# rrahn/libspm

Hardware: AMD Instinct MI355X
Metric: Gbases/s scanned, Myers k<=3 |P|=100 (higher is better)
Workload: dtype u32

## Files before the change

### libspm_amd/csrc/common.hpp

```cpp
#pragma once

#include <hip/hip_runtime.h>

#include <algorithm>
#include <cstdint>
#include <functional>
#include <cstdio>
#include <string>
#include <utility>
#include <vector>

#include "../../include/spm_hip.h"
#include "scan_plan.hpp"

namespace spm_hip
{

constexpr int kWave = 64;

struct error_sink
{
    std::string msg;
};

extern thread_local std::string g_init_error;

}

struct hits_block
{
    spm_hit *d_hits = nullptr;
    unsigned long long *d_count = nullptr;
    uint64_t cap = 0;
    hipEvent_t ev[4] = {nullptr, nullptr, nullptr, nullptr};
    bool zeroed = false;
    unsigned long long *h_c = nullptr;
    hipEvent_t ev_done = nullptr;
};

struct spm_ctx
{
    int device = 0;
    hipStream_t stream = nullptr;
    bool own_stream = false;
    int n_cu = 256;
    std::string err;
    void *d_scratch = nullptr;
    size_t scratch_bytes = 0;
    std::vector<hits_block> pool;
    std::vector<std::pair<void *, uint64_t>> jst_pool;
    ulonglong2 *d_band_tab = nullptr;
    uint64_t band_slots = 0;
    bool band_dirty = false;
    uint32_t *d_table_poison = nullptr;
    uint8_t *h_stage = nullptr;
    size_t stage_half = 0;
    hipEvent_t stage_ev[2] = {nullptr, nullptr};
    unsigned long long *h_counters = nullptr;
};

struct spm_text
{
    spm_ctx *ctx = nullptr;
    uint8_t *d = nullptr;
    uint64_t n = 0;
    uint64_t alloc = 0;
    uint32_t sigma = 4;
    bool owned = false;
    uint32_t *d_packed = nullptr;
    uint64_t packed_words = 0;
};

struct spm_hits : hits_block
{
    spm_ctx *ctx = nullptr;
    uint64_t cand_cap = 0;
    uint64_t band_cap = 0;
    uint64_t n = 0;
    bool counted = false;
    bool hook_final = false;
    unsigned long long fan_count = 0;
    bool sorted_host = false;
    std::vector<spm_hit> host;
    spm_scan_stats stats{};
    bool timed = false;
    void *d_aux[2] = {nullptr, nullptr};
    bool pending = false;
    bool c_on_the_way = false;
    bool d_count_cleared = false;
    const spm_text *d_text = nullptr;
    const struct spm_patterns *d_patterns = nullptr;
    uint64_t d_begin = 0, d_end = 0;
    spm_scan_opts d_opts{};
    const spm_text *al_text = nullptr;
    const struct spm_patterns *al_patterns = nullptr;
    uint64_t al_lo = 0;
    uint64_t al_pos_offset = 0;
    bool al_stateful = false;
    bool al_device_segs = false;
    std::vector<uint64_t> al_segs;
};

inline void hits_adopt(spm_hits &h, spm_hits &from)
{
    std::swap(static_cast<hits_block &>(h), static_cast<hits_block &>(from));
    std::swap(h.h_c, from.h_c);
    std::swap(h.ev_done, from.ev_done);
    std::swap(h.d_aux, from.d_aux);
    from.d_count_cleared = h.d_count_cleared;
    h.d_count_cleared = false;
    h.n = from.n;
    h.counted = from.counted;
    h.stats = from.stats;
    h.cand_cap = from.cand_cap;
    h.band_cap = from.band_cap;
    h.timed = from.timed;
    h.sorted_host = false;
    h.host.clear();
}

#define SPM_TRY(call)                                                                                                  \
    do {                                                                                                               \
        const int _rc = (call);                                                                                        \
        if (_rc != SPM_OK)                                                                                             \
            return _rc;                                                                                                \
    } while (0)

struct pass_entry
{
    const uint4 *ht;
    uint32_t ht_mask;
    uint32_t pad;
};

struct dev_scratch
{
    std::vector<void *> owned;
    template <typename T>
    hipError_t alloc(T **p, size_t bytes)
    {
        const hipError_t e = hipMalloc(reinterpret_cast<void **>(p), bytes);
        if (e == hipSuccess)
            owned.push_back(*p);
        return e;
    }
    ~dev_scratch()
    {
        for (void *p : owned)
            hipFree(p);
    }
};

#define SPM_SET_ERR(ctx, ...)                                                                                          \
    do {                                                                                                               \
        char _b[512];                                                                                                  \
        snprintf(_b, sizeof(_b), __VA_ARGS__);                                                                         \
        if (ctx)                                                                                                       \
            (ctx)->err = _b;                                                                                           \
        else                                                                                                           \
            spm_hip::g_init_error = _b;                                                                                \
    } while (0)

#define SPM_HIP_CHECK(ctx, call)                                                                                       \
    do {                                                                                                               \
        hipError_t _e = (call);                                                                                        \
        if (_e != hipSuccess) {                                                                                        \
            SPM_SET_ERR(ctx, "%s failed: %s (%s:%d)", #call, hipGetErrorString(_e), __FILE__, __LINE__);               \
            return SPM_E_HIP;                                                                                          \
        }                                                                                                              \
    } while (0)
```

### libspm_amd/csrc/filter.hpp

```cpp
#pragma once

#include "brute.hpp"
#include "common.hpp"
#include "filter_shared.hpp"
#include "pack.hpp"
#include "hd.hpp"

namespace spm_hip
{

struct survivor
{
    uint32_t key;
    uint32_t t_lo, t_hi;
    uint32_t pad;
};
constexpr uint32_t kSurvInvalid = 0xFFFFFFFFu;

struct band_rec
{
    uint32_t slot;
    uint32_t val;
    uint32_t seg;
    uint32_t band;
// ... 996 lines not shown
        return (uint32_t)(W.hi >> (2 * (first - 32)));
    return (uint32_t)(W.lo >> (2 * first)) | (first ? (uint32_t)(W.hi << (2 * (32 - first)) ) : 0u);
}

__device__ __forceinline__ bool seed_sig_ok(const text64 &W, uint32_t sig, uint32_t r, uint32_t n, uint32_t H)
{
    if (n == 0)
        return true;
    const uint32_t rb = r < 16 ? r : 16;
    const uint32_t nl = rb < n ? rb : n;
    uint32_t got = nl ? syms16(W, 16 - rb) : 0u;
    if (nl < 16) {
        got &= (1u << (2 * nl)) - 1;
        got |= syms16(W, 16 + H) << (2 * nl);
    }
    const uint32_t mask = n >= 16 ? 0xFFFFFFFFu : ((1u << (2 * n)) - 1);
    return ((got ^ sig) & mask) == 0;
}

constexpr uint32_t kPairCap = 128;
struct pair_queue
{
    uint32_t t_lo[kPairCap], t_hi[kPairCap], val[kPairCap], rng[kPairCap], seg[kPairCap];
};
struct band_queue
{
    uint32_t key_lo[kPairCap], key_hi[kPairCap], run_lo[kPairCap], run_hi[kPairCap];
    uint32_t elect[128];
};

struct band_chunk
{
    uint64_t base;
    uint32_t used, size, draws;
};
constexpr uint32_t kDenseDraws = 4;

__device__ __forceinline__ void insert_bands(const resolve_params &R, band_queue &B, uint32_t first, uint32_t n,
                                             uint32_t lane, band_chunk &C)
{
    bool act = lane < n;
    unsigned long long bkey = 0, run = 0;
    if (act)
        bkey = ((unsigned long long)B.key_hi[first + lane] << 32) | B.key_lo[first + lane];
    if (!R.overlap) {
        const uint32_t h = (uint32_t)mix64(bkey) & 127u;
        if (act)
            B.elect[h] = lane;
        __builtin_amdgcn_fence(__ATOMIC_RELEASE, "wavefront");
        __builtin_amdgcn_wave_barrier();
        const uint32_t w = act ? B.elect[h] : lane;
        const unsigned long long wkey = ((unsigned long long)B.key_hi[first + w] << 32) | B.key_lo[first + w];
        const bool follower = act && w != lane && wkey == bkey;
        if (follower) {
            atomicOr(&B.run_lo[first + w], B.run_lo[first + lane]);
            atomicOr(&B.run_hi[first + w], B.run_hi[first + lane]);
            act = false;
        }
        __builtin_amdgcn_fence(__ATOMIC_RELEASE, "wavefront");
        __builtin_amdgcn_wave_barrier();
    }
    if (act)
        run = ((unsigned long long)B.run_hi[first + lane] << 32) | B.run_lo[first + lane];
    bool claimed = false;
    uint32_t s2 = (uint32_t)mix64(bkey) & R.table_mask;
    if (act) {
        bool placed = false;
        for (uint32_t tries = 0; tries < 8192 && !placed; ++tries) {
            if ((tries & 31u) == 31u && __hip_atomic_load(&R.counters[kCntVoid], __ATOMIC_RELAXED, __HIP_MEMORY_SCOPE_AGENT) != 0)
                break;
            const unsigned long long o = atomicCAS(&R.band_tab[s2].x, kBandEmpty, bkey);
            if (o == kBandEmpty) {
                claimed = true;
                placed = true;
            } else if (o == bkey) {
                placed = true;
            } else {
                s2 = (s2 + 1) & R.table_mask;
            }
        }
        if (!placed) {
            atomicAdd(&R.counters[kCntVoid], 1ull);
            *R.table_poison = 1u;
        }
        else if (R.overlap)
            atomicAdd(&R.band_tab[s2].y, 1ull);
        else
            atomicAnd(&R.band_tab[s2].y, ~run);
    }
    const uint64_t mm = __ballot(claimed);
    if (mm == 0)
        return;
    const uint32_t nn = __popcll(mm);
    if (C.used + nn > C.size) {
        for (uint32_t q = C.used + lane; q < C.size; q += 64)
            if (C.base + q < R.band_cap)
                R.bands[C.base + q].val = kBandInvalid;
        uint32_t next = C.size * 2 < kChunkMin ? kChunkMin : (C.size * 2 > kChunkMax ? kChunkMax : C.size * 2);
        next = next < nn ? nn : next;
        if (C.draws < kDenseDraws) {
            next = nn;
            ++C.draws;
        }
        unsigned long long b = 0;
        if (lane == 0)
            b = atomicAdd(&R.counters[kCntBandSlots], (unsigned long long)next);
        C.base = ((uint64_t)(uint32_t)__builtin_amdgcn_readfirstlane((uint32_t)(b >> 32)) << 32) |
                 (uint32_t)__builtin_amdgcn_readfirstlane((uint32_t)b);
        C.used = 0;
        C.size = next;
    }
    if (claimed) {
        const uint64_t idx = C.base + C.used + __popcll(mm & ((1ull << lane) - 1));
        if (idx < R.band_cap) {
            band_rec br;
            br.slot = s2;
            br.val = (uint32_t)(bkey >> 43) << 11;
            br.seg = (uint32_t)((bkey & ((1ull << 43) - 1)) >> R.band_bits);
            br.band = (uint32_t)(bkey & ((1ull << R.band_bits) - 1));
            R.bands[idx] = br;
        } else {
            atomicAdd(&R.counters[kCntVoid], 1ull);
            *R.table_poison = 1u;
        }
    }
    C.used += nn;
}

__device__ __forceinline__ unsigned long long wave_reserve_hits(unsigned long long *counter, uint32_t mine)
{
    const uint32_t lane = threadIdx.x & 63;
    uint32_t incl = mine;
#pragma unroll
    for (int o = 1; o < 64; o <<= 1) {
        const uint32_t up = (uint32_t)__shfl_up((int)incl, o);
        if (lane >= (uint32_t)o)
            incl += up;
    }
    const uint32_t total = (uint32_t)__shfl((int)incl, 63);
    unsigned long long base = 0;
    if (total != 0) {
        if (lane == 0)
            base = atomicAdd(counter, (unsigned long long)total);
        base = ((unsigned long long)(uint32_t)__builtin_amdgcn_readfirstlane((uint32_t)(base >> 32)) << 32) |
               (uint32_t)__builtin_amdgcn_readfirstlane((uint32_t)base);
    }
    return base + (incl - mine);
}

__device__ __forceinline__ bool seen_insert_raw(unsigned long long *seen, uint32_t seen_mask, unsigned long long *overflow,
                                                uint32_t pat, int64_t e)
{
    const unsigned long long key = ((unsigned long long)pat << 40) | (unsigned long long)e;
    uint32_t slot = (uint32_t)(mix64(key)) & seen_mask;
    for (uint32_t tries = 0; tries < 64; ++tries) {
        if (tries == 4 && __hip_atomic_load(overflow, __ATOMIC_RELAXED, __HIP_MEMORY_SCOPE_AGENT) != 0)
            return false;
        const unsigned long long old = atomicCAS(&seen[slot], ~0ull, key);
        if (old == ~0ull)
            return true;
        if (old == key)
            return false;
        slot = (slot + 1) & seen_mask;
    }
    atomicAdd(overflow, 1ull);
    return false;
}

struct resolve_wave
{
    pair_queue *Q;
    band_queue *B;
    uint32_t qn, bn;
    band_chunk C;
    uint32_t n_cand;
};

__device__ __forceinline__ void queue_sync()
{
    __builtin_amdgcn_fence(__ATOMIC_RELEASE, "wavefront");
    __builtin_amdgcn_wave_barrier();
}

__device__ __forceinline__ void check_pairs(const resolve_params &R, resolve_wave &S, uint32_t n, uint32_t lane)
{
    pair_queue &Q = *S.Q;
    band_queue &B = *S.B;
    S.qn -= n;
    const uint32_t first = S.qn;
    bool live = lane < n;
    uint64_t t = 0, seg = 0;
    uint32_t val = 0, rng = 0;
    int64_t sb = (int64_t)R.hay_begin, se = (int64_t)R.hay_end;
    if (live) {
        const uint32_t i = first + lane;
        t = ((uint64_t)Q.t_hi[i] << 32) | Q.t_lo[i];
        val = Q.val[i];
        rng = Q.rng[i];
        seg = Q.seg[i];
        if (R.seg_offsets) {
            sb = (int64_t)R.seg_offsets[seg];
            se = (int64_t)R.seg_offsets[seg + 1];
        }
    }
    queue_sync();
    bool through = live;
    const uint32_t pat = val >> 11;
    if (live && !(rng & kRngRun)) {
        if (!(rng & kSeedChecked)) {
            live = seed_intact(R, t, val, (rng >> 16) & 0x1F, (rng & kRngWhole) ? R.key_len + ((rng >> 5) & 0x1F) : 0u, sb, se);
            rng |= kSeedChecked;
        }
        through = live;
        if (live && R.pieces_check) {
            const uint32_t m = (uint32_t)R.m[pat], k = (uint32_t)R.k[pat];
            if (pieces_apply(R, t, val, m, k, sb, se)) {
                const uint32_t v = pieces_visit(R, t, val, rng, m, k);
                live = v != 0;
                through = v == 2;
            }
        }
    }
    {
        const bool back = live && !through;
        const uint64_t mm = __ballot(back);
        if (back) {
            const uint32_t q = S.qn + __popcll(mm & ((1ull << lane) - 1));
            Q.t_lo[q] = (uint32_t)t;
            Q.t_hi[q] = (uint32_t)(t >> 32);
            Q.val[q] = val;
            Q.rng[q] = rng;
            Q.seg[q] = (uint32_t)seg;
        }
        S.qn += __popcll(mm);
    }
    int64_t b_cur = 0, b_last = -1, d_lo = 0, d_hi = 0;
    if (R.exact_hits) {
        bool fresh = false;
        int64_t e = 0;
        if (live && through) {
            ++S.n_cand;
            e = (int64_t)t - (int64_t)(val & 0x7FF) + (int64_t)R.m[pat];
            int64_t own_b = (int64_t)R.scan_begin, own_e = (int64_t)R.scan_end;
            if (R.seg_offsets) {
                own_b = R.seg_owned ? sb + (int64_t)R.seg_owned[seg] : sb;
                own_e = se;
            }
            fresh = e >= own_b + 1 && e <= own_e && (!R.seen || seen_insert_raw(R.seen, R.seen_mask, R.overflow, pat, e));
        }
        const unsigned long long idx = wave_reserve_hits(R.hit_counter, fresh ? 1u : 0u);
        if (fresh && idx < R.hit_cap) {
            spm_hit h;
            h.pos = (R.report_begin ? (uint64_t)(e - (int64_t)R.m[pat]) : (uint64_t)e) + R.pos_offset;
            h.pattern = pat;
            h.score = 0;
            R.hits[idx] = h;
        }
        queue_sync();
        return;
    }
    if (live && through) {
        ++S.n_cand;
        d_hi = (int64_t)t - (int64_t)(val & 0x7FF) - sb + (int64_t)R.max_m;
        d_lo = d_hi - (int64_t)((rng & kRngRun) ? (rng & 0x7FF) : 0u);
        b_cur = d_lo / (int64_t)R.Bw;
        b_last = d_hi / (int64_t)R.Bw;
        if (R.overlap && b_cur > 0 && d_lo - b_cur * (int64_t)R.Bw <= (int64_t)R.k[pat])
            --b_cur;
        if ((uint64_t)b_last >> R.band_bits) {
            atomicAdd(&R.counters[kCntVoid], 1ull);
            b_last = b_cur - 1;
        }
    }
    for (;;) {
        const bool have = b_cur <= b_last;
        const uint64_t mm = __ballot(have);
        if (mm == 0)
            break;
        if (have) {
            const unsigned long long bkey =
                ((unsigned long long)pat << 43) | ((unsigned long long)seg << R.band_bits) | (unsigned long long)b_cur;
            const int64_t b0 = b_cur * (int64_t)R.Bw;
            const uint32_t o_lo = (uint32_t)(d_lo > b0 ? d_lo - b0 : 0);
            const uint32_t o_hi = (uint32_t)(d_hi < b0 + (int64_t)R.Bw - 1 ? d_hi - b0 : (int64_t)R.Bw - 1);
            const unsigned long long run = (o_hi - o_lo >= 63 ? ~0ull : ((1ull << (o_hi - o_lo + 1)) - 1)) << o_lo;
            const uint32_t q = S.bn + __popcll(mm & ((1ull << lane) - 1));
            B.key_lo[q] = (uint32_t)bkey;
            B.key_hi[q] = (uint32_t)(bkey >> 32);
            B.run_lo[q] = (uint32_t)run;
            B.run_hi[q] = (uint32_t)(run >> 32);
        }
        S.bn += __popcll(mm);
        queue_sync();
        if (S.bn >= 64) {
            S.bn -= 64;
            insert_bands(R, B, S.bn, 64, lane, S.C);
            queue_sync();
        }
        ++b_cur;
    }
    queue_sync();
}

__global__ __launch_bounds__(256) void resolve_kernel(const resolve_params R)
{
    __shared__ pair_queue pair_queues[4];
    __shared__ band_queue band_queues[4];
    unsigned long long n = R.counters[kCntSurvSlots];
    if (blockIdx.x == 0 && threadIdx.x == 0) {
        atomicAdd(&R.counters[kCntUnreadSurvSum], n);
        atomicMax(&R.counters[kCntUnreadSurvMax], n);
    }
    if (n > R.surv_cap)
        n = R.surv_cap;
    if (!R.exact_hits && __hip_atomic_load(R.table_poison, __ATOMIC_RELAXED, __HIP_MEMORY_SCOPE_AGENT) != 0) {
        if (blockIdx.x == 0 && threadIdx.x == 0)
            atomicAdd(&R.counters[kCntVoid], 1ull);
        return;
    }
    const uint32_t lane = threadIdx.x & 63;
    resolve_wave S;
    S.Q = &pair_queues[threadIdx.x >> 6];
    S.B = &band_queues[threadIdx.x >> 6];
    S.qn = 0;
    S.bn = 0;
    S.C.base = 0;
    S.C.used = 0;
    S.C.size = 0;
    S.C.draws = 0;
    S.n_cand = 0;
    pair_queue &Q = *S.Q;
    const uint64_t stride = (uint64_t)gridDim.x * blockDim.x;
    const uint64_t rounds = (n + stride - 1) / stride;
    for (uint64_t r = 0; r < rounds; ++r) {
        if ((r & 7u) == 7u &&
            __builtin_amdgcn_readfirstlane((uint32_t)(__hip_atomic_load(&R.counters[kCntVoid], __ATOMIC_RELAXED, __HIP_MEMORY_SCOPE_AGENT) != 0)))
            break;
        const uint64_t i = r * stride + (uint64_t)blockIdx.x * blockDim.x + threadIdx.x;
        bool probing = false;
        uint32_t key = 0;
        uint64_t t = 0, seg = 0;
        pass_entry T = R.passes[0];
        if (i < n) {
            const survivor sv = R.surv[i];
            if (sv.t_hi != kSurvInvalid) {
                probing = true;
                key = sv.key;
                t = ((uint64_t)sv.t_hi << 32) | sv.t_lo;
                if (sv.pad != 0)
                    T = R.passes[sv.pad];
            }
        }
        if (probing && R.seg_offsets) {
            uint64_t lo = 0, hi = R.n_segments;
            while (hi - lo > 1) {
                const uint64_t mid = (lo + hi) >> 1;
                if (R.seg_offsets[mid] <= t)
                    lo = mid;
                else
                    hi = mid;
            }
            seg = lo;
            if ((int64_t)t + (int64_t)R.key_len > (int64_t)R.seg_offsets[lo + 1])
                probing = false;
        }
        text64 W;
        W.lo = 0;
        W.hi = 0;
        W.ok = false;
        if (probing && R.flank_check) {
            int64_t sb = (int64_t)R.hay_begin, se = (int64_t)R.hay_end;
            if (R.seg_offsets) {
                sb = (int64_t)R.seg_offsets[seg];
                se = (int64_t)R.seg_offsets[seg + 1];
            }
            if ((int64_t)t - 16 >= sb && (int64_t)t + 48 <= se && t + 48 <= R.text_alloc) {
                const uint8_t *p = R.text + (t - 16);
                W.lo = (uint64_t)pack16(load_bytes16(p)) | ((uint64_t)pack16(load_bytes16(p + 16)) << 32);
                W.hi = (uint64_t)pack16(load_bytes16(p + 32)) | ((uint64_t)pack16(load_bytes16(p + 48)) << 32);
                W.ok = true;
            }
        }
        uint32_t first = 0, cnt = 0;
        {
            uint32_t slot = ht_hash(key) & T.ht_mask;
            while (__ballot(probing) != 0) {
                if (probing) {
                    const uint4 d = T.ht[slot];
                    if (d.z == 0) {
                        probing = false;
                    } else if (d.x == key) {
                        first = d.y;
                        cnt = d.z;
                        probing = false;
                    } else {
                        slot = (slot + 1) & T.ht_mask;
                    }
                }
            }
        }
        uint32_t incl = cnt;
#pragma unroll
        for (int o = 1; o < 64; o <<= 1) {
            const uint32_t up = (uint32_t)__shfl_up((int)incl, o);
            if (lane >= (uint32_t)o)
                incl += up;
        }
        const uint32_t total = (uint32_t)__builtin_amdgcn_readfirstlane(__shfl((int)incl, 63));
        for (uint32_t p0 = 0; p0 < total; p0 += 64) {
            const uint32_t i = p0 + lane;
            bool have = i < total;
            uint32_t owner = 0;
#pragma unroll
            for (int step = 32; step > 0; step >>= 1) {
                const uint32_t v = (uint32_t)__shfl((int)incl, (int)(owner + step - 1));
                if (v <= i)
                    owner += step;
            }
            owner = owner > 63 ? 63 : owner;
            const uint32_t o_incl = (uint32_t)__shfl((int)incl, (int)owner), o_cnt = (uint32_t)__shfl((int)cnt, (int)owner);
            const uint32_t o_first = (uint32_t)__shfl((int)first, (int)owner);
            const uint64_t o_t = ((uint64_t)(uint32_t)__shfl((int)(uint32_t)(t >> 32), (int)owner) << 32) |
                                 (uint32_t)__shfl((int)(uint32_t)t, (int)owner);
            const uint32_t o_seg = (uint32_t)__shfl((int)(uint32_t)seg, (int)owner);
            text64 OW;
            OW.lo = ((uint64_t)(uint32_t)__shfl((int)(uint32_t)(W.lo >> 32), (int)owner) << 32) |
                    (uint32_t)__shfl((int)(uint32_t)W.lo, (int)owner);
            OW.hi = ((uint64_t)(uint32_t)__shfl((int)(uint32_t)(W.hi >> 32), (int)owner) << 32) |
                    (uint32_t)__shfl((int)(uint32_t)W.hi, (int)owner);
            OW.ok = __shfl((int)W.ok, (int)owner) != 0;
            uint32_t val = 0, rng = 0;
            if (have) {
                const uint4 e = R.entries[o_first + (i - (o_incl - o_cnt))];
                val = e.x;
                rng = e.z;
                if (!(rng & kRngRun)) {
                    const uint32_t r0 = rng & 0x1F, ns = (rng >> 5) & 0x1F;
                    const bool whole = (rng & kRngWhole) != 0;
                    rng = (r0 << 16) | (whole ? (ns << 5) | kRngWhole : 0u);
                    if (OW.ok) {
                        if (!seed_sig_ok(OW, e.y, r0, ns, R.key_len))
                            have = false;
                        else if (whole)
                            rng |= kSeedChecked;
                    }
                }
            }
            const uint64_t mm = __ballot(have);
            if (mm != 0) {
                if (have) {
                    const uint32_t q = S.qn + __popcll(mm & ((1ull << lane) - 1));
                    Q.t_lo[q] = (uint32_t)o_t;
                    Q.t_hi[q] = (uint32_t)(o_t >> 32);
                    Q.val[q] = val;
                    Q.rng[q] = rng;
                    Q.seg[q] = o_seg;
                }
                S.qn += __popcll(mm);
                queue_sync();
                while (S.qn >= 64)
                    check_pairs(R, S, 64, lane);
            }
        }
    }
    while (S.qn != 0)
        check_pairs(R, S, S.qn < 64 ? S.qn : 64, lane);
    if (S.bn != 0)
        insert_bands(R, *S.B, 0, S.bn, lane, S.C);
    for (uint32_t q = S.C.used + lane; q < S.C.size; q += 64)
        if (S.C.base + q < R.band_cap)
            R.bands[S.C.base + q].val = kBandInvalid;
    wave_count_add(R.counters + kCntPairs, S.n_cand);
}

__device__ __forceinline__ bool seen_insert(const verify_params &P, uint32_t pat, int64_t e)
{
    return seen_insert_raw(P.seen, P.seen_mask, P.overflow, pat, e);
}

__global__ __launch_bounds__(256) void band_select_kernel(const verify_params P, band_rec *out, unsigned long long *out_count)
{
    unsigned long long n = P.counters[kCntBandSlots];
    if (n > P.band_cap)
        n = P.band_cap;
    const uint32_t lane = threadIdx.x & 63;
    const uint64_t stride = (uint64_t)gridDim.x * blockDim.x;
    const uint64_t rounds = (n + stride - 1) / stride;
    for (uint64_t r = 0; r < rounds; ++r) {
        const uint64_t i = r * stride + (uint64_t)blockIdx.x * blockDim.x + threadIdx.x;
        bool keep = false;
        band_rec c;
        c.val = kBandInvalid;
        if (i < n) {
            c = P.bands[i];
            if (c.val != kBandInvalid) {
                const uint32_t cnt = (uint32_t)band_value(P.band_tab[c.slot].y, true);
                band_release(P.band_tab, c.slot);
                keep = cnt >= (P.surplus ? (uint32_t)P.surplus[c.val >> 11] : 1u);
            }
        }
        const uint64_t m = __ballot(keep);
        if (m != 0) {
            unsigned long long base = 0;
            const int leader = __ffsll((unsigned long long)m) - 1;
            if ((int)lane == leader)
                base = atomicAdd(out_count, (unsigned long long)__popcll(m));
            base = __shfl(base, leader);
            if (keep)
                out[base + __popcll(m & ((1ull << lane) - 1))] = c;
        }
    }
}

constexpr uint32_t kRunAnalysed = 0x400u;
constexpr uint32_t kRunFollower = 0x200u;
constexpr uint32_t kRunLenShift = 5, kRunLenMask = 0x3u, kRunHiMask = 0x1Fu;
constexpr uint32_t kRunTouchLeft = 0x80u, kRunTouchRight = 0x100u;
constexpr uint32_t kRunMax = 4;
constexpr uint32_t kHitStage = 192;

__device__ __forceinline__ uint32_t band_lookup(const verify_params &P, unsigned long long bkey)
{
    uint32_t s2 = (uint32_t)mix64(bkey) & P.table_mask;
    for (uint32_t tries = 0; tries < 8192; ++tries) {
        const unsigned long long o = P.band_tab[s2].x;
        if (o == bkey)
            return s2;
        if (o == kBandEmpty)
            return 0xFFFFFFFFu;
        s2 = (s2 + 1) & P.table_mask;
    }
    return 0xFFFFFFFFu;
}

__global__ __launch_bounds__(256) void band_runs_kernel(const verify_params P, band_rec *bands, band_rec *heads,
                                                        unsigned long long *head_count)
{
    __shared__ uint32_t wave_tot01[4], wave_tot23[4];
    __shared__ unsigned long long chunk_base;
    unsigned long long n = P.counters[P.band_counter];
    if (n > P.band_cap)
        n = P.band_cap;
    constexpr uint32_t PER = 8;
    const uint32_t tid = threadIdx.x, lane = tid & 63, wave = tid >> 6;
    for (uint64_t c0 = (uint64_t)blockIdx.x * (256 * PER); c0 < n; c0 += (uint64_t)gridDim.x * (256 * PER)) {
        band_rec mine[PER];
        uint32_t head_mask = 0, cnt = 0;
#pragma unroll
        for (uint32_t j = 0; j < PER; ++j) {
            const uint64_t i = c0 + (uint64_t)j * 256 + tid;
            mine[j].val = kBandInvalid;
            if (i >= n)
                continue;
            band_rec c = bands[i];
            if (c.val == kBandInvalid)
                continue;
            const unsigned long long base = ((unsigned long long)(c.val >> 11) << 43) | ((unsigned long long)c.seg << P.band_bits);
            uint32_t code = kRunAnalysed;
            const bool pred = c.band > 0 && band_lookup(P, base | (unsigned long long)(c.band - 1)) != 0xFFFFFFFFu;
            if (c.band % kRunMax != 0 && pred) {
                code |= kRunFollower;
            } else {
                uint32_t followers = 0, last = c.slot;
                bool cut = true;
                for (uint32_t r = 1; r < kRunMax && (c.band + r) % kRunMax != 0; ++r) {
                    const uint32_t s2 = band_lookup(P, base | (unsigned long long)(c.band + r));
                    if (s2 == 0xFFFFFFFFu) {
                        cut = false;
                        break;
                    }
                    followers = r;
                    last = s2;
                }
                const bool succ = cut && band_lookup(P, base | (unsigned long long)(c.band + followers + 1)) != 0xFFFFFFFFu;
                const unsigned long long v = band_value(P.band_tab[last].y, false);
                const uint32_t hi = v ? (uint32_t)(63 - __clzll((long long)v)) : 0u;
                code |= (followers << kRunLenShift) | (hi & kRunHiMask) | (pred ? kRunTouchLeft : 0u) | (succ ? kRunTouchRight : 0u);
                head_mask |= 1u << j;
                ++cnt;
            }
            c.val = (c.val & ~0x7FFu) | code;
            mine[j] = c;
        }
        uint32_t c01 = 0, c23 = 0;
#pragma unroll
        for (uint32_t j = 0; j < PER; ++j)
            if (head_mask & (1u << j)) {
                const uint32_t cls = (mine[j].val >> kRunLenShift) & kRunLenMask;
                const uint32_t one = 1u << (16 * (cls & 1u));
                c01 += cls < 2 ? one : 0u;
                c23 += cls < 2 ? 0u : one;
            }
        uint32_t i01 = c01, i23 = c23;
#pragma unroll
        for (int o = 1; o < 64; o <<= 1) {
            const uint32_t u01 = (uint32_t)__shfl_up((int)i01, o), u23 = (uint32_t)__shfl_up((int)i23, o);
            if (lane >= (uint32_t)o) {
                i01 += u01;
                i23 += u23;
            }
        }
        if (lane == 63) {
            wave_tot01[wave] = i01;
            wave_tot23[wave] = i23;
        }
        __syncthreads();
        uint32_t off01 = 0, off23 = 0, tot01 = 0, tot23 = 0;
        for (uint32_t w = 0; w < 4; ++w) {
            off01 += w < wave ? wave_tot01[w] : 0u;
            off23 += w < wave ? wave_tot23[w] : 0u;
// ... 491 lines not shown
```

### libspm_amd/csrc/hits.hip

```cpp
#include "internal.hpp"
#include "hd.hpp"

static int hits_count(spm_hits *h)
{
    spm_ctx *ctx = h->ctx;
    if (h->pending) {
        const int rc = spm_complete_deferred(h);
        if (rc != SPM_OK)
            return rc;
    }
    if (!h->counted) {
        unsigned long long *c = ctx->h_counters;
        SPM_HIP_CHECK(ctx, hipMemcpyAsync(c, h->d_count, kCntReadBackCount * sizeof(unsigned long long), hipMemcpyDeviceToHost, ctx->stream));
        SPM_HIP_CHECK(ctx, hipStreamSynchronize(ctx->stream));
        h->n = c[kCntHits];
        h->counted = true;
    }
    if (h->n > h->cap) {
        SPM_SET_ERR(ctx, "scan produced %llu hits but the buffer holds %llu; raise spm_scan_opts.max_hits",
                    (unsigned long long)h->n, (unsigned long long)h->cap);
        return SPM_E_OVERFLOW;
    }
    return SPM_OK;
}

extern "C" int spm_hip_hits_view(spm_hits *h, const spm_hit **records, uint64_t *n)
{
    if (!h || !records || !n)
        return SPM_E_INVALID;
    int rc = hits_count(h);
    if (rc != SPM_OK)
        return rc;
    if (!h->sorted_host) {
        h->host.resize(h->n);
        if (h->n) {
            SPM_HIP_CHECK(h->ctx, hipMemcpyAsync(h->host.data(), h->d_hits, h->n * sizeof(spm_hit),
                                                 hipMemcpyDeviceToHost, h->ctx->stream));
            SPM_HIP_CHECK(h->ctx, hipStreamSynchronize(h->ctx->stream));
        }
        std::sort(h->host.begin(), h->host.end(), [](const spm_hit &a, const spm_hit &b) {
            return a.pattern != b.pattern ? a.pattern < b.pattern : (int64_t)a.pos < (int64_t)b.pos;
        });
        h->sorted_host = true;
    }
    *records = h->host.data();
    *n = h->n;
    return SPM_OK;
}

extern "C" int spm_hip_hits_device(spm_hits *h, const void **device_records, uint64_t *n)
{
    if (!h || !device_records || !n)
        return SPM_E_INVALID;
    int rc = hits_count(h);
    if (rc != SPM_OK)
        return rc;
    *device_records = h->d_hits;
    *n = h->n;
    return SPM_OK;
}

extern "C" int spm_hip_hits_copy_device(spm_hits *h, void *device_dst, uint64_t cap, uint64_t *n)
{
    if (!h || !n || (cap && !device_dst))
        return SPM_E_INVALID;
    int rc = hits_count(h);
    if (rc != SPM_OK)
        return rc;
    *n = h->n;
    const uint64_t c = std::min(h->n, cap);
    if (c)
        SPM_HIP_CHECK(h->ctx, hipMemcpyAsync(device_dst, h->d_hits, c * sizeof(spm_hit), hipMemcpyDeviceToDevice,
                                             h->ctx->stream));
    return SPM_OK;
}

__global__ __launch_bounds__(256) void hits_fused_copy_kernel(uint4 *__restrict__ dst, const uint4 *__restrict__ src,
                                                                unsigned long long n, unsigned long long n_copy)
{
    const uint64_t i = (uint64_t)blockIdx.x * blockDim.x + threadIdx.x;
    if (i == 0)
        dst[0] = make_uint4((uint32_t)n, (uint32_t)(n >> 32), 0u, 0u);
    for (uint64_t r = i; r < n_copy; r += (uint64_t)gridDim.x * blockDim.x)
        dst[1 + r] = src[r];
}

extern "C" int spm_hip_hits_copy_fused(spm_hits *h, void *device_dst, uint64_t cap, uint64_t *n)
{
    if (!h || !n || !device_dst)
        return SPM_E_INVALID;
    int rc = hits_count(h);
    if (rc != SPM_OK)
        return rc;
    *n = h->n;
    if ((uintptr_t)device_dst & 15) {
        SPM_SET_ERR(h->ctx, "spm_hip_hits_copy_fused: the destination must be 16-byte aligned");
        return SPM_E_INVALID;
    }
    const uint64_t c = std::min(h->n, cap);
    const unsigned grid = (unsigned)std::max<uint64_t>(1, std::min<uint64_t>((c + 255) / 256, (uint64_t)h->ctx->n_cu * 4));
    hipLaunchKernelGGL(hits_fused_copy_kernel, dim3(grid), dim3(256), 0, h->ctx->stream, static_cast<uint4 *>(device_dst),
                       reinterpret_cast<const uint4 *>(h->d_hits), (unsigned long long)h->n, (unsigned long long)c);
    SPM_HIP_CHECK(h->ctx, hipGetLastError());
    return SPM_OK;
}

__global__ __launch_bounds__(256) void hits_fused_copy_device_kernel(uint4 *__restrict__ dst, const uint4 *__restrict__ src,
                                                                       unsigned long long *__restrict__ counters,
                                                                       unsigned long long *__restrict__ host_c,
                                                                       unsigned long long cap, unsigned long long hit_cap,
                                                                       unsigned long long cand_cap)
{
    const unsigned long long n = counters[kCntHits];
    const unsigned long long status = scan_needs_host(counters, cand_cap, n, hit_cap) ? 1ull : 0ull;
    const unsigned long long n_copy = n < cap ? (n < hit_cap ? n : hit_cap) : cap;
    const uint64_t i = (uint64_t)blockIdx.x * blockDim.x + threadIdx.x;
    if (i == 0)
        dst[0] = make_uint4((uint32_t)n, (uint32_t)(n >> 32), (uint32_t)status, 0u);
    if (blockIdx.x == 0 && threadIdx.x < kCntReadBack && host_c)
        host_c[threadIdx.x] = counters[threadIdx.x];
    for (uint64_t r = i; r < n_copy; r += (uint64_t)gridDim.x * blockDim.x)
        dst[1 + r] = src[r];
    if (host_c) {
        __syncthreads();
        __shared__ unsigned int last;
        if (threadIdx.x == 0) {
            __threadfence();
            last = atomicAdd(&counters[kCntTicket], 1ull) == (unsigned long long)gridDim.x - 1 ? 1u : 0u;
        }
        __syncthreads();
        if (last && threadIdx.x < kCntBlock)
            counters[threadIdx.x] = 0;
    }
}

extern "C" int spm_hip_hits_copy_fused_device(spm_hits *h, void *device_dst, uint64_t cap)
{
    if (!h || !device_dst || ((uintptr_t)device_dst & 15))
        return SPM_E_INVALID;
    if (h->pending && h->c_on_the_way) {
        const int rc = hits_count(h);
        if (rc != SPM_OK && rc != SPM_E_OVERFLOW)
            return rc;
    }
    if (!h->pending && h->counted) {
        const uint64_t c = std::min(h->n, std::min<uint64_t>(cap, h->cap));
        const unsigned g1 = (unsigned)std::max<uint64_t>(1, std::min<uint64_t>((c + 255) / 256, (uint64_t)h->ctx->n_cu * 4));
        hipLaunchKernelGGL(hits_fused_copy_kernel, dim3(g1), dim3(256), 0, h->ctx->stream, static_cast<uint4 *>(device_dst),
                           reinterpret_cast<const uint4 *>(h->d_hits), (unsigned long long)h->n, (unsigned long long)c);
        SPM_HIP_CHECK(h->ctx, hipGetLastError());
        return SPM_OK;
    }
    const unsigned grid = (unsigned)std::max<uint64_t>(1, std::min<uint64_t>((std::min<uint64_t>(cap, h->cap) + 255) / 256, (uint64_t)h->ctx->n_cu));
    unsigned long long *host_c = h->pending ? h->h_c : nullptr;
    hipLaunchKernelGGL(hits_fused_copy_device_kernel, dim3(grid), dim3(256), 0, h->ctx->stream, static_cast<uint4 *>(device_dst),
                       reinterpret_cast<const uint4 *>(h->d_hits), h->d_count, host_c, (unsigned long long)cap,
                       (unsigned long long)h->cap, (unsigned long long)(h->cand_cap ? h->cand_cap : ~0ull));
    SPM_HIP_CHECK(h->ctx, hipGetLastError());
    if (host_c) {
        SPM_HIP_CHECK(h->ctx, hipEventRecord(h->ev_done, h->ctx->stream));
        h->c_on_the_way = true;
        h->d_count_cleared = true;
    }
    return SPM_OK;
}

extern "C" int spm_hip_hits_stats(const spm_hits *hc, spm_scan_stats *out)
{
    if (!hc || !out)
        return SPM_E_INVALID;
    spm_hits *h = const_cast<spm_hits *>(hc);
    int rc = hits_count(h);
    if (rc != SPM_OK && rc != SPM_E_OVERFLOW)
        return rc;
    if (h->timed) {
        SPM_HIP_CHECK(h->ctx, hipEventSynchronize(h->ev[3]));
        hipEventElapsedTime(&h->stats.ms_total, h->ev[0], h->ev[3]);
        hipEventElapsedTime(&h->stats.ms_main, h->ev[1], h->ev[2]);
        hipEventElapsedTime(&h->stats.ms_verify, h->ev[2], h->ev[3]);
    }
    h->stats.n_hits = h->n;
    *out = h->stats;
    return SPM_OK;
}

extern "C" uint64_t spm_hip_hits_checksum(spm_hits *h)
{
    const spm_hit *r = nullptr;
    uint64_t n = 0;
    if (spm_hip_hits_view(h, &r, &n) != SPM_OK)
        return 0;
    uint64_t s = 0;
    for (uint64_t i = 0; i < n; ++i)
        s += mix64(r[i].pos ^ ((uint64_t)r[i].pattern << 40) ^ ((uint64_t)(uint32_t)r[i].score << 58));
    return s;
}

extern "C" void spm_hip_hits_destroy(spm_hits *h)
{
    if (!h)
        return;
    if (h->pending)
        (void)spm_complete_deferred(h);
    if (h->d_aux[0] || h->d_aux[1]) {
        if (h->ctx)
            hipStreamSynchronize(h->ctx->stream);
        hipFree(h->d_aux[0]);
        hipFree(h->d_aux[1]);
    }
    if (h->ctx && h->d_hits && h->d_count && h->ev[3] && h->ctx->pool.size() < 8) {
        hits_block b = *h;
        b.zeroed = h->d_count_cleared || hipMemsetAsync(b.d_count, 0, kCntBlock * sizeof(unsigned long long), h->ctx->stream) == hipSuccess;
        h->ctx->pool.push_back(b);
    } else {
        if (h->ctx)
            hipStreamSynchronize(h->ctx->stream);
        hipFree(h->d_hits);
        hipFree(h->d_count);
        for (int i = 0; i < 4; ++i)
            if (h->ev[i])
                hipEventDestroy(h->ev[i]);
        if (h->h_c)
            hipHostFree(h->h_c);
        if (h->ev_done)
            hipEventDestroy(h->ev_done);
    }
    delete h;
}


void spm_warm_hits_kernels()
{
    hipFuncAttributes a;
    (void)hipFuncGetAttributes(&a, (const void *)hits_fused_copy_kernel);
}
```

### libspm_amd/csrc/internal.hpp

```cpp
#pragma once

#include <algorithm>
#include <chrono>
#include <cmath>
#include <cstdlib>
#include <cstring>
#include <memory>

#include "common.hpp"
#include "index_build.hpp"

using namespace spm_hip;

struct spm_patterns : spm_hip::seed_index
{
    spm_ctx *ctx = nullptr;
    int algo = 0;
    uint32_t n = 0;
    uint32_t sigma = 4;
    std::vector<uint8_t> ranks;
    std::vector<uint32_t> offsets;
    std::vector<int32_t> m, k;
    uint32_t n_groups = 0;
    uint32_t max_m = 0;
    uint32_t max_window = 0;
    uint32_t max_k = 0;
    uint32_t NW = 1;
    bool is_myers() const { return algo == SPM_ALGO_MYERS || algo == SPM_ALGO_MYERS_PREFIX; }
    void *d_arena = nullptr;
    uint32_t *d_peq = nullptr;
    uint32_t *d_peq_bot = nullptr;
    uint32_t *d_peq_verify = nullptr;
    uint32_t *d_hp0 = nullptr;
    int32_t *d_m = nullptr;
    int32_t *d_k = nullptr;
    mutable uint64_t cand_hint = 0;
    uint8_t *d_surplus = nullptr;
    uint8_t *d_ranks = nullptr;
    uint32_t *d_offsets = nullptr;
    uint32_t *d_needle_pk = nullptr;
    uint32_t *d_pk_offsets = nullptr;
    uint16_t *d_seed_q = nullptr;
    pass_entry *d_pass_tab = nullptr;
    uint4 *d_entries = nullptr;
    mutable uint64_t hit_hint = 0;
    mutable bool scanned = false;
    mutable int exact_whole = -1;
    mutable uint64_t band_hint = 0;
    spm_build_stats build{};
    mutable void *d_align = nullptr;
    mutable const uint64_t *d_al_rpeq = nullptr;
    mutable const uint32_t *d_al_rpeq_off = nullptr;
    mutable const uint8_t *d_al_ranks = nullptr;
    mutable const uint32_t *d_al_offsets = nullptr;
};

using clk = std::chrono::steady_clock;
inline float ms_since(clk::time_point t) { return std::chrono::duration<float, std::milli>(clk::now() - t).count(); }
inline bool spm_trace_on()
{
    const char *v = getenv("SPM_HIP_TRACE");
    return v && *v && *v != '0';
}


struct scan_tuning
{
    int cand_cap = 0;
    int brute_cutoff = 1;
    int verify_wave_min_words = 8;
    int span_budget = 0;
    int verify_runs = 1;
    int verify_runs_min_bands = 65536;
    int band_cap = 0;
    static scan_tuning from_env()
    {
        scan_tuning T;
        T.cand_cap = env_int("SPM_HIP_FILTER_CAND_CAP", 0);
        T.brute_cutoff = env_int("SPM_HIP_BRUTE_CUTOFF", 1);
        T.verify_wave_min_words = env_int("SPM_HIP_VERIFY_WAVE_MIN_WORDS", 8);
        T.span_budget = env_int("SPM_HIP_FILTER_SPAN_BUDGET", 0);
        T.verify_runs = env_int("SPM_HIP_VERIFY_RUNS", 1);
        T.verify_runs_min_bands = env_int("SPM_HIP_VERIFY_RUNS_MIN_BANDS", 65536);
        T.band_cap = env_int("SPM_HIP_FILTER_BAND_CAP", 0);
        return T;
    }
};

struct scan_args
{
    spm_ctx *ctx;
    const spm_text *text;
    uint64_t begin, end, ctx_begin;
    const spm_patterns *ps;
    spm_scan_opts opts;
    spm_hits *hits;
    scan_tuning tune;
    const uint64_t *seg_offsets = nullptr;
    uint64_t n_segments = 0;
    const uint64_t *d_seg_offsets = nullptr;
    const uint32_t *d_seg_owned = nullptr;
};

struct scan_state
{
    retry_state retry;
    filter_result filt;
    const uint64_t *segs = nullptr;
    std::vector<uint64_t> seg_host;
    const std::vector<uint64_t> *tiles = nullptr;
};

void state_to_internal(const spm_patterns *p, const void *state, std::vector<uint32_t> &out);
void state_from_internal(const spm_patterns *p, const std::vector<uint32_t> &in, void *state);
int text_alloc(spm_ctx *ctx, uint64_t n, uint32_t sigma, spm_text **out);
int ensure_scratch(spm_ctx *ctx, size_t bytes);
int run_brute(const scan_args &A, const scan_state &S, uint64_t begin, uint64_t end, uint64_t ctx_begin,
              const uint32_t *d_state_in, uint32_t *d_state_out, bool report, bool single_tile);
int run_filter(const scan_args &A, const retry_state &R, filter_result &out);
int scan_impl(spm_ctx *ctx, const spm_text *text, uint64_t begin, uint64_t end, const spm_patterns *patterns,
              const spm_scan_opts *opts_in, const void *state_in, void *state_out, const uint64_t *seg_offsets,
              uint64_t n_segments, spm_hits **out, const uint64_t *d_seg_offsets = nullptr,
              const uint32_t *d_seg_owned = nullptr, const std::function<int(spm_hits *)> *after_launch = nullptr);

struct align_work
{
    const spm_patterns *ps = nullptr;
    const spm_text *text = nullptr;
    uint64_t pos_offset = 0;
    const spm_hit *hits = nullptr;
    uint64_t n = 0;
    const uint64_t *lo = nullptr;
    const uint32_t *cig_off = nullptr;
    bool begin_only = false;
    spm_aln *d_recs = nullptr;
    uint32_t *d_ops = nullptr;
    uint64_t n_ops = 0;
    spm_aln *h_recs = nullptr;
    uint32_t *h_ops = nullptr;
    const char *who = "";
};
int align_run(spm_ctx *ctx, const align_work &W, spm_align_stats &stats);

void spm_warm_text_kernels();
void spm_warm_brute_kernels();
void spm_warm_filter_kernels();
void spm_warm_hits_kernels();
void spm_warm_jst_kernels();
void spm_warm_align_kernels();

int spm_complete_deferred(spm_hits *h);
```

### libspm_amd/csrc/patterns.hip

```cpp
#include "internal.hpp"
#include "tables_build.hpp"

namespace
{
struct needle_upload
{
    struct item
    {
        void **dst;
        const void *src;
        size_t bytes, off;
    };
    std::vector<item> items;
    size_t total = 0;
    size_t add(void **dst, const void *src, size_t bytes, size_t zero_tail = 0)
    {
        items.push_back(item{dst, src, bytes, total});
        total += (std::max<size_t>(bytes + zero_tail, 16) + 255) & ~(size_t)255;
        return items.size() - 1;
    }
    hipError_t place(void **arena)
    {
        hipError_t e = hipMalloc(arena, std::max<size_t>(total, 256));
        if (e != hipSuccess)
            return e;
        for (item &it : items)
            *it.dst = static_cast<uint8_t *>(*arena) + it.off;
        return hipSuccess;
    }
    void fill(uint8_t *out, size_t lo, size_t hi) const
    {
        memset(out, 0, hi - lo);
        size_t i = std::upper_bound(items.begin(), items.end(), lo, [](size_t v, const item &it) { return v < it.off; }) - items.begin();
        i = i ? i - 1 : 0;
        for (; i < items.size() && items[i].off < hi; ++i) {
            const item &it = items[i];
            const size_t a = std::max(lo, it.off), b = std::min(hi, it.off + it.bytes);
            if (a < b && it.src)
                memcpy(out + (a - lo), static_cast<const uint8_t *>(it.src) + (a - it.off), b - a);
        }
    }
    hipError_t stream(spm_ctx *ctx, void *arena, unsigned n_threads) const
    {
        const size_t half = ctx->stage_half;
        std::unique_ptr<thread_team> team;
        if (total > 4 * half && n_threads > 1)
            team.reset(new thread_team(std::min(n_threads, 8u)));
        hipError_t e = hipSuccess;
        unsigned c = 0;
        for (size_t lo = 0; lo < total && e == hipSuccess; lo += half, ++c) {
            const size_t hi = std::min(total, lo + half);
            uint8_t *h = ctx->h_stage + (c & 1) * half;
            if (c >= 2)
                e = hipEventSynchronize(ctx->stage_ev[c & 1]);
            if (e != hipSuccess)
                break;
            if (team)
                team->run((hi - lo + 65535) / 65536, [&](size_t b0, size_t b1, unsigned) {
                    const size_t a = lo + b0 * 65536, b = std::min(hi, lo + b1 * 65536);
                    if (a < b)
                        fill(h + (a - lo), a, b);
                });
            else
                fill(h, lo, hi);
            e = hipMemcpyAsync(static_cast<uint8_t *>(arena) + lo, h, hi - lo, hipMemcpyHostToDevice, ctx->stream);
            if (e == hipSuccess)
                e = hipEventRecord(ctx->stage_ev[c & 1], ctx->stream);
        }
        if (e == hipSuccess)
            e = hipStreamSynchronize(ctx->stream);
        return e;
    }
};
}

extern "C" int spm_hip_patterns_create(spm_ctx *ctx, int algo, const uint8_t *ranks_concat, const uint32_t *offsets,
                                       uint32_t n_patterns, const uint16_t *k, uint32_t sigma, spm_patterns **out)
{
    if (!ctx || !out || (n_patterns && (!offsets || !ranks_concat)) || sigma < 2 || sigma > 255 || algo < 0 ||
        algo > SPM_ALGO_HORSPOOL) {
        SPM_SET_ERR(ctx, "spm_hip_patterns_create: invalid argument");
        return SPM_E_INVALID;
    }
    SPM_HIP_CHECK(ctx, hipSetDevice(ctx->device));
    const auto t_begin = clk::now();
    std::unique_ptr<spm_patterns, void (*)(spm_patterns *)> ps(new spm_patterns, spm_hip_patterns_destroy);
    ps->ctx = ctx;
    ps->algo = algo;
    ps->n = n_patterns;
    ps->sigma = sigma;
    ps->offsets.assign(offsets, offsets + n_patterns + 1);
    ps->ranks.assign(ranks_concat, ranks_concat + (n_patterns ? offsets[n_patterns] : 0));
    ps->n_groups = std::max(1u, (n_patterns + 63) / 64);
    ps->m.assign((size_t)ps->n_groups * 64, 0);
    ps->k.assign((size_t)ps->n_groups * 64, -1);
    for (uint32_t p = 0; p < n_patterns; ++p) {
        if (offsets[p + 1] < offsets[p]) {
            SPM_SET_ERR(ctx, "spm_hip_patterns_create: offsets not ascending");
            return SPM_E_INVALID;
        }
        const uint32_t m = offsets[p + 1] - offsets[p];
        if (m > SPM_MAX_NEEDLE) {
            SPM_SET_ERR(ctx, "needle %u has %u symbols; limit is %u", p, m, SPM_MAX_NEEDLE);
            return SPM_E_UNSUPPORTED;
        }
        const uint32_t kk = (ps->is_myers() && k) ? k[p] : 0;
        ps->m[p] = (int32_t)m;
        ps->k[p] = (int32_t)kk;
        ps->max_m = std::max(ps->max_m, m);
        ps->max_k = std::max(ps->max_k, kk);
        ps->max_window = std::max(ps->max_window, m + kk);
    }
    ps->NW = next_pow2(std::max(1u, (ps->max_m + 31) / 32));
    const uint32_t NW = ps->NW;
    const index_tuning tune = index_tuning::from_env();
    ps->build.threads = tune.n_threads();
    needle_view nv;
    nv.algo = algo;
    nv.n = n_patterns;
    nv.sigma = sigma;
    nv.ranks = ps->ranks.data();
    nv.offsets = ps->offsets.data();
    nv.m = ps->m.data();
    nv.k = ps->k.data();
    nv.max_k = ps->max_k;
    needle_upload up;
    auto upload = [&](auto **dst, const void *src, size_t bytes) -> hipError_t {
        up.add(reinterpret_cast<void **>(dst), src, bytes);
        return hipSuccess;
    };
    double ms_upload = 0;
    long pass_tab_item = -1;
    std::vector<uint32_t> pk, pk_off;
    std::vector<uint8_t> surplus;
    auto t0 = clk::now();

    brute_tables bt;
    {
        build_brute_tables(nv, ps->n_groups, NW, sigma <= 5 || sigma == 15, tune.n_threads(), bt);
        ps->build.ms_tables = ms_since(t0);
        SPM_HIP_CHECK(ctx, upload(&ps->d_peq, bt.peq.data(), bt.peq.size() * sizeof(uint32_t)));
        if (!bt.verify.empty())
            SPM_HIP_CHECK(ctx, upload(&ps->d_peq_verify, bt.verify.data(), bt.verify.size() * sizeof(uint32_t)));
        if (!bt.bot.empty())
            SPM_HIP_CHECK(ctx, upload(&ps->d_peq_bot, bt.bot.data(), bt.bot.size() * sizeof(uint32_t)));
        if (!bt.hp0.empty())
            SPM_HIP_CHECK(ctx, upload(&ps->d_hp0, bt.hp0.data(), bt.hp0.size() * sizeof(uint32_t)));
        SPM_HIP_CHECK(ctx, upload(&ps->d_m, ps->m.data(), ps->m.size() * sizeof(int32_t)));
        SPM_HIP_CHECK(ctx, upload(&ps->d_k, ps->k.data(), ps->k.size() * sizeof(int32_t)));
    }

    if ((sigma == 4 || sigma == 5 || sigma == 15) && algo != SPM_ALGO_MYERS_PREFIX && n_patterns > 0) {
        const auto ti = clk::now();
        int rc = build_filter_index(nv, tune, *ps);
        if (rc != SPM_OK)
            return rc;
        ps->build.ms_index = ms_since(ti);
        if (!ps->fidx.empty()) {
            for (filter_index &F : ps->fidx) {
                SPM_HIP_CHECK(ctx, upload(&F.d_bitmap, F.h_image.data(), F.h_image.size() * sizeof(uint32_t)));
                SPM_HIP_CHECK(ctx, upload(&F.d_ht, F.h_ht.data(), F.h_ht.size() * sizeof(u32x4)));
                if (!F.h_buckets.empty())
                    SPM_HIP_CHECK(ctx, upload(&F.d_buckets, F.h_buckets.data(), F.h_buckets.size() * sizeof(uint16_t)));
                ps->build.keys += F.n_keys;
                for (uint32_t d = 0; d < 16; ++d)
                    ps->build.anchor_sixteenths += (F.dimer_set >> d) & 1u;
            }
            pass_tab_item = (long)up.add(reinterpret_cast<void **>(&ps->d_pass_tab), nullptr, ps->fidx.size() * sizeof(pass_entry));
            SPM_HIP_CHECK(ctx, upload(&ps->d_entries, ps->h_entries.data(), ps->h_entries.size() * sizeof(u32x4)));
            up.add(reinterpret_cast<void **>(&ps->d_ranks), ps->ranks.data(), ps->ranks.size(), 64);
            SPM_HIP_CHECK(ctx, upload(&ps->d_offsets, ps->offsets.data(), ps->offsets.size() * sizeof(uint32_t)));
            if (ps->sigma == 4) {
                pack_needles(nv, pk, pk_off, tune.n_threads());
                SPM_HIP_CHECK(ctx, upload(&ps->d_needle_pk, pk.data(), pk.size() * sizeof(uint32_t)));
                SPM_HIP_CHECK(ctx, upload(&ps->d_pk_offsets, pk_off.data(), pk_off.size() * sizeof(uint32_t)));
            }
            SPM_HIP_CHECK(ctx, upload(&ps->d_seed_q, ps->seed_q.data(), ps->seed_q.size() * sizeof(uint16_t)));
        }
        if (!ps->fidx.empty() && ps->max_k >= kMergeMinK && ps->max_k <= 1000) {
            surplus.assign(ps->m.size(), 1);
            for (uint32_t p = 0; p < ps->n; ++p)
                surplus[p] = (uint8_t)(ps->seed_n[p] - (uint32_t)ps->k[p]);
            SPM_HIP_CHECK(ctx, upload(&ps->d_surplus, surplus.data(), surplus.size()));
        }
    }
    {
        const auto tu = clk::now();
        SPM_HIP_CHECK(ctx, up.place(&ps->d_arena));
        const double ms_place = ms_since(tu);
        std::vector<pass_entry> pt;
        for (filter_index &F : ps->fidx)
            pt.push_back(pass_entry{reinterpret_cast<const uint4 *>(F.d_ht), F.ht_mask, 0});
        if (pass_tab_item >= 0)
            up.items[(size_t)pass_tab_item].src = pt.data();
        SPM_HIP_CHECK(ctx, up.stream(ctx, ps->d_arena, tune.n_threads()));
        for (filter_index &F : ps->fidx) {
            F.h_image = std::vector<uint32_t>();
            F.h_ht = std::vector<u32x4>();
            F.h_buckets = std::vector<uint16_t>();
        }
        ps->h_entries = std::vector<u32x4>();
        ps->build.bytes_device = up.total;
        ms_upload = ms_since(tu);
        if (spm_trace_on())
            fprintf(stderr, "[spm_hip] patterns_create: one allocation of %.2f MiB in %.2f ms, streamed up in %.2f ms\n",
                    up.total / 1048576.0, ms_place, ms_upload - ms_place);
    }
    ps->build.ms_upload = (float)ms_upload;
    ps->build.ms_total = ms_since(t_begin);
    ps->build.passes = (uint32_t)ps->fidx.size();
    ps->build.dense = ps->filter_dense ? 1u : 0u;
    ps->build.stride = ps->filter_stride;
    ps->build.key_len = ps->filter_key_len;
    if (spm_trace_on())
        fprintf(stderr, "[spm_hip] patterns_create: %u needles, algo %d, sigma %u -> %u pass(es)%s, %llu keys, %u/16 of the dimers; "
                        "%.2f ms (tables %.2f, index %.2f, upload %.2f; %u threads)\n",
                n_patterns, algo, sigma, ps->build.passes, ps->build.dense ? " dense" : "", (unsigned long long)ps->build.keys,
                ps->build.anchor_sixteenths, ps->build.ms_total, ps->build.ms_tables, ps->build.ms_index, ps->build.ms_upload,
                ps->build.threads);
    *out = ps.release();
    return SPM_OK;
}

extern "C" int spm_hip_patterns_build_stats(const spm_patterns *p, spm_build_stats *out)
{
    if (!p || !out)
        return SPM_E_INVALID;
    *out = p->build;
    return SPM_OK;
}

extern "C" void spm_hip_patterns_destroy(spm_patterns *p)
{
    if (!p)
        return;
    hipFree(p->d_arena);
    hipFree(p->d_align);
    delete p;
}

extern "C" uint64_t spm_hip_patterns_window_size(const spm_patterns *p, uint32_t pattern)
{
    if (!p || pattern >= p->n || p->m[pattern] == 0)
        return 0;
    return (uint64_t)p->m[pattern] + (p->is_myers() ? (uint64_t)p->k[pattern] : 0);
}

extern "C" int spm_hip_patterns_filterable(const spm_patterns *p) { return p && !p->fidx.empty() ? 1 : 0; }

static uint32_t abi_words(const spm_patterns *p)
{
    return p->is_myers() ? std::max(1u, (p->max_m + 63) / 64) : std::max(1u, (p->max_m + 31) / 32);
}

extern "C" size_t spm_hip_patterns_state_stride(const spm_patterns *p)
{
    if (!p)
        return 0;
    const uint32_t nw = abi_words(p);
    return p->is_myers() ? 8 + (size_t)16 * nw : 8 + (size_t)4 * ((nw + 1) & ~1u);
}

static void set_bits(std::vector<uint32_t> &v, uint32_t lo, uint32_t hi)
{
    for (uint32_t b = lo; b < hi; ++b)
        v[b / 32] |= 1u << (b % 32);
}

extern "C" int spm_hip_patterns_state_init(const spm_patterns *p, void *state)
{
    if (!p || !state)
        return SPM_E_INVALID;
    const size_t stride = spm_hip_patterns_state_stride(p);
    const uint32_t nw = abi_words(p);
    memset(state, 0, stride * p->n);
    for (uint32_t i = 0; i < p->n; ++i) {
        uint8_t *rec = (uint8_t *)state + stride * i;
        const uint32_t m = (uint32_t)p->m[i];
        if (p->is_myers()) {
            int32_t score = (int32_t)m;
            memcpy(rec, &score, 4);
            memcpy(rec + 4, &nw, 4);
            uint64_t *vp = (uint64_t *)(rec + 8);
            for (uint32_t b = 0; b < m; ++b)
                vp[b / 64] |= 1ull << (b % 64);
        } else {
            memcpy(rec, &nw, 4);
            uint32_t *r = (uint32_t *)(rec + 8);
            for (uint32_t w = 0; w < nw; ++w)
                r[w] = 0xFFFFFFFFu;
        }
    }
    return SPM_OK;
}

void state_to_internal(const spm_patterns *p, const void *state, std::vector<uint32_t> &out)
{
    const uint32_t NW = p->NW, nw = abi_words(p);
    const size_t stride = spm_hip_patterns_state_stride(p);
    const uint32_t rows = p->is_myers() ? 2 * NW + 1 : NW;
    out.assign((size_t)p->n_groups * rows * 64, 0);
    for (uint32_t i = 0; i < p->n_groups * 64; ++i) {
        const uint32_t g = i / 64, l = i % 64;
        const uint32_t m = i < p->n ? (uint32_t)p->m[i] : 0;
        const uint32_t off = NW * 32 - m;
        auto at = [&](uint32_t row) -> uint32_t & { return out[((size_t)g * rows + row) * 64 + l]; };
        if (i >= p->n || m == 0) {
            if (p->is_myers())
                at(2 * NW) = 0x3FFFFFFF;
            else
                for (uint32_t w = 0; w < NW; ++w)
                    at(w) = 0xFFFFFFFFu;
            continue;
        }
        const uint8_t *rec = (const uint8_t *)state + stride * i;
        if (p->is_myers()) {
            int32_t score;
            memcpy(&score, rec, 4);
            const uint64_t *vp = (const uint64_t *)(rec + 8);
            const uint64_t *vn = vp + nw;
            for (uint32_t j = 0; j < m; ++j) {
                const uint32_t b = off + j;
                if ((vp[j / 64] >> (j % 64)) & 1)
                    at(b / 32) |= 1u << (b % 32);
                if ((vn[j / 64] >> (j % 64)) & 1)
                    at(NW + b / 32) |= 1u << (b % 32);
            }
            at(2 * NW) = (uint32_t)score;
        } else {
            const uint32_t *r = (const uint32_t *)(rec + 8);
            for (uint32_t w = 0; w < NW; ++w)
                at(w) = 0;
            for (uint32_t j = 0; j < m; ++j) {
                const uint32_t b = off + j;
                if ((r[j / 32] >> (j % 32)) & 1)
                    at(b / 32) |= 1u << (b % 32);
            }
        }
    }
}

void state_from_internal(const spm_patterns *p, const std::vector<uint32_t> &in, void *state)
{
    const uint32_t NW = p->NW, nw = abi_words(p);
    const size_t stride = spm_hip_patterns_state_stride(p);
    const uint32_t rows = p->is_myers() ? 2 * NW + 1 : NW;
    memset(state, 0, stride * p->n);
    for (uint32_t i = 0; i < p->n; ++i) {
        const uint32_t g = i / 64, l = i % 64;
        const uint32_t m = (uint32_t)p->m[i];
        const uint32_t off = NW * 32 - m;
        auto at = [&](uint32_t row) -> uint32_t { return in[((size_t)g * rows + row) * 64 + l]; };
        uint8_t *rec = (uint8_t *)state + stride * i;
        if (p->is_myers()) {
            int32_t score = m ? (int32_t)at(2 * NW) : 0;
            memcpy(rec, &score, 4);
            memcpy(rec + 4, &nw, 4);
            uint64_t *vp = (uint64_t *)(rec + 8);
            uint64_t *vn = vp + nw;
            for (uint32_t j = 0; j < m; ++j) {
                const uint32_t b = off + j;
                if ((at(b / 32) >> (b % 32)) & 1)
                    vp[j / 64] |= 1ull << (j % 64);
                if ((at(NW + b / 32) >> (b % 32)) & 1)
                    vn[j / 64] |= 1ull << (j % 64);
            }
        } else {
            memcpy(rec, &nw, 4);
            uint32_t *r = (uint32_t *)(rec + 8);
            for (uint32_t w = 0; w < nw; ++w)
                r[w] = 0xFFFFFFFFu;
            for (uint32_t j = 0; j < m; ++j) {
                const uint32_t b = off + j;
                if (!((at(b / 32) >> (b % 32)) & 1))
                    r[j / 32] &= ~(1u << (j % 32));
            }
        }
    }
}

extern "C" int spm_hip_host_selftest(int algo, const uint8_t *ranks_concat, const uint32_t *offsets, uint32_t n_patterns,
                                     const uint16_t *k, uint32_t sigma, uint64_t *stats)
{
    return spm_hip::host_selftest(algo, ranks_concat, offsets, n_patterns, k, sigma, stats);
}
```

### libspm_amd/csrc/scan.hip

```cpp
#include "internal.hpp"
#include "filter_shared.hpp"

int ensure_scratch(spm_ctx *ctx, size_t bytes)
{
    if (ctx->scratch_bytes >= bytes)
        return SPM_OK;
    const auto t0 = clk::now();
    if (ctx->d_scratch) {
        SPM_HIP_CHECK(ctx, hipStreamSynchronize(ctx->stream));
        SPM_HIP_CHECK(ctx, hipFree(ctx->d_scratch));
        ctx->d_scratch = nullptr;
        ctx->scratch_bytes = 0;
    }
    size_t want = bytes + bytes / 4;
    hipError_t e = hipMalloc(&ctx->d_scratch, want);
    if (e != hipSuccess) {
        (void)hipGetLastError();
        want = bytes;
        SPM_HIP_CHECK(ctx, hipMalloc(&ctx->d_scratch, want));
    }
    ctx->scratch_bytes = want;
    if (spm_trace_on())
        fprintf(stderr, "[spm_hip] scratch (survivor / band lists, dedupe set) grows to %.1f MiB: %.2f ms\n", want / 1048576.0, ms_since(t0));
    return SPM_OK;
}

extern "C" int spm_hip_scan(spm_ctx *ctx, const spm_text *text, uint64_t begin, uint64_t end,
                            const spm_patterns *patterns, const spm_scan_opts *opts_in, const void *state_in,
                            void *state_out, spm_hits **out)
{
    return scan_impl(ctx, text, begin, end, patterns, opts_in, state_in, state_out, nullptr, 0, out);
}

extern "C" int spm_hip_scan_segments(spm_ctx *ctx, const spm_text *text, const uint64_t *seg_offsets,
                                     uint64_t n_segments, const spm_patterns *patterns, const spm_scan_opts *opts_in,
                                     spm_hits **out)
{
    if (!ctx || !text || !seg_offsets || n_segments == 0) {
        SPM_SET_ERR(ctx, "spm_hip_scan_segments: invalid argument");
        return SPM_E_INVALID;
    }
    for (uint64_t s = 0; s < n_segments; ++s)
        if (seg_offsets[s + 1] < seg_offsets[s] || seg_offsets[s + 1] > text->n) {
            SPM_SET_ERR(ctx, "spm_hip_scan_segments: offsets must ascend and stay inside the text");
            return SPM_E_INVALID;
        }
    spm_scan_opts o{};
    if (opts_in)
        o = *opts_in;
    o.left_context = 0;
    return scan_impl(ctx, text, seg_offsets[0], seg_offsets[n_segments], patterns, &o, nullptr, nullptr, seg_offsets,
                     n_segments, out);
}

namespace
{
int acquire_hits(spm_ctx *ctx, spm_hits *H)
{
    for (size_t i = 0; i < ctx->pool.size(); ++i)
        if (ctx->pool[i].cap == H->cap) {
            static_cast<hits_block &>(*H) = ctx->pool[i];
            ctx->pool.erase(ctx->pool.begin() + i);
            if (!H->zeroed)
                SPM_HIP_CHECK(ctx, hipMemsetAsync(H->d_count, 0, kCntBlock * sizeof(unsigned long long), ctx->stream));
            return SPM_OK;
        }
    const auto ta = clk::now();
    SPM_HIP_CHECK(ctx, hipMalloc(&H->d_hits, std::max<uint64_t>(H->cap, 1) * sizeof(spm_hit)));
    if (spm_trace_on())
        fprintf(stderr, "[spm_hip] a new hit buffer (%llu records): %.2f ms\n", (unsigned long long)H->cap, ms_since(ta));
    SPM_HIP_CHECK(ctx, hipMalloc(&H->d_count, kCntBlock * sizeof(unsigned long long)));
    for (int i = 0; i < 4; ++i)
        SPM_HIP_CHECK(ctx, hipEventCreate(&H->ev[i]));
    SPM_HIP_CHECK(ctx, hipMemsetAsync(H->d_count, 0, kCntBlock * sizeof(unsigned long long), ctx->stream));
    return SPM_OK;
}

int choose_engine(spm_ctx *ctx, const spm_patterns *patterns, const spm_scan_opts &opts, uint64_t range, bool stateful,
                  bool segmented, uint64_t state_prefix, bool &use_filter)
{
    const bool want_filter = opts.engine == SPM_ENGINE_FILTER || (opts.engine == SPM_ENGINE_AUTO && !patterns->fidx.empty());
    if (opts.engine == SPM_ENGINE_FILTER && patterns->fidx.empty()) {
        SPM_SET_ERR(ctx, "spm_hip_scan: the seed filter does not apply to this needle set");
        return SPM_E_UNSUPPORTED;
    }
    use_filter = want_filter && patterns->n > 0 && range > 0;
    if (stateful && use_filter &&
        (segmented || range <= state_prefix || (opts.engine != SPM_ENGINE_FILTER && range < (1u << 18))))
        use_filter = false;
    if (opts.engine == SPM_ENGINE_FILTER && !use_filter && patterns->n > 0 && range > 0) {
        SPM_SET_ERR(ctx, "spm_hip_scan: the seed filter does not apply to this stateful scan (chunk shorter than a window)");
        return SPM_E_UNSUPPORTED;
    }
    return SPM_OK;
}

void take_stats(spm_hits *h, const unsigned long long *c)
{
    h->stats.n_candidates = c[kCntPairs];
    h->stats.n_bands = (uint32_t)std::min<unsigned long long>(c[kCntBandsVerified], 0xFFFFFFFFull);
}

struct scan_call
{
    const scan_args &A;
    spm_ctx *ctx;
    const spm_patterns *ps;
    spm_hits *H;
    uint64_t begin, end;
    const void *state_in;
    void *state_out;
    bool has_state, stateful, segmented;
    uint64_t state_prefix, tail_begin;
    const std::function<int(spm_hits *)> *after_launch;
    scan_state S{};

    int finish_trivial()
    {
        SPM_HIP_CHECK(ctx, hipEventRecord(H->ev[1], ctx->stream));
        SPM_HIP_CHECK(ctx, hipEventRecord(H->ev[2], ctx->stream));
        SPM_HIP_CHECK(ctx, hipEventRecord(H->ev[3], ctx->stream));
        H->stats.engine_used = SPM_ENGINE_BRUTE;
        if (state_in && state_out && state_out != state_in)
            memcpy(state_out, state_in, spm_hip_patterns_state_stride(ps) * ps->n);
        else if (state_out && !state_in)
            spm_hip_patterns_state_init(ps, state_out);
        return SPM_OK;
    }

    int clear_counters(bool forget_launches = true)
    {
        SPM_HIP_CHECK(ctx, hipMemsetAsync(H->d_count, 0, kCntBlock * sizeof(unsigned long long), ctx->stream));
        if (forget_launches)
            H->stats.main_launches = 0;
        return SPM_OK;
    }

    int host_segments()
    {
        if (S.segs || !A.d_seg_offsets)
            return SPM_OK;
        S.seg_host.resize(A.n_segments + 1);
        SPM_HIP_CHECK(ctx, hipMemcpyAsync(S.seg_host.data(), A.d_seg_offsets, (A.n_segments + 1) * sizeof(uint64_t),
                                          hipMemcpyDeviceToHost, ctx->stream));
        SPM_HIP_CHECK(ctx, hipStreamSynchronize(ctx->stream));
        S.segs = S.seg_host.data();
        return SPM_OK;
    }

    int defer_completion()
    {
        if (!H->h_c)
            SPM_HIP_CHECK(ctx, hipHostMalloc(&H->h_c, kCntBlock * sizeof(unsigned long long), hipHostMallocDefault));
        if (!H->ev_done)
            SPM_HIP_CHECK(ctx, hipEventCreateWithFlags(&H->ev_done, hipEventDisableTiming));
        H->pending = true;
        H->c_on_the_way = false;
        H->d_count_cleared = false;
        ctx->band_dirty = false;
        H->d_text = A.text;
        H->d_patterns = ps;
        H->d_begin = begin;
        H->d_end = end;
        H->d_opts = A.opts;
        return SPM_OK;
    }

    int span_fallback(unsigned long long *c)
    {
        const uint64_t n_ovf = c[kCntSpansGaveUp];
        std::vector<uint64_t> ov(2 * n_ovf);
        SPM_HIP_CHECK(ctx, hipMemcpyAsync(ov.data(), S.filt.d_ovf, ov.size() * sizeof(uint64_t), hipMemcpyDeviceToHost, ctx->stream));
        SPM_HIP_CHECK(ctx, hipStreamSynchronize(ctx->stream));
        const fallback_plan F = plan_fallback(ov.data(), n_ovf, A.begin, end, ps->max_window, (uint64_t)ctx->n_cu, ps->n_groups);
        if (segmented)
            SPM_TRY(host_segments());
        std::vector<uint64_t> tab;
        fallback_tiles(F, A.ctx_begin, segmented ? S.segs : nullptr, A.n_segments, tab);
        H->stats.fallback_spans = (uint32_t)std::min<uint64_t>(n_ovf, 0xFFFFFFFFu);
        if (!tab.empty()) {
            if (tab.size() / 3 > 0xFFFFFFFFull) {
                SPM_SET_ERR(ctx, "span-local fallback: too many tiles");
                return SPM_E_UNSUPPORTED;
            }
            S.tiles = &tab;
            const int rc = run_brute(A, S, begin, end, A.ctx_begin, nullptr, nullptr, true, false);
            S.tiles = nullptr;
            SPM_TRY(rc);
            H->stats.main_launches--;
            SPM_HIP_CHECK(ctx, hipEventRecord(H->ev[3], ctx->stream));
            SPM_HIP_CHECK(ctx, hipMemcpyAsync(c, H->d_count, kCntReadBackRescan * sizeof(unsigned long long), hipMemcpyDeviceToHost, ctx->stream));
            SPM_HIP_CHECK(ctx, hipStreamSynchronize(ctx->stream));
        }
        H->stats.fallback_symbols = F.total;
        return SPM_OK;
    }

    int filter_attempts(bool &use_filter, bool &deferred)
    {
        unsigned long long *c = ctx->h_counters;
        for (int round = 0, attempt = 0; round < 3;) {
            SPM_TRY(run_filter(A, S.retry, S.filt));
            H->cand_cap = S.filt.cand_cap;
            H->band_cap = S.filt.band_cap;
            if ((A.opts.flags & SPM_SCAN_DEFER) && round == 0 && attempt == 0 && !stateful && !segmented && !after_launch) {
                deferred = true;
                return defer_completion();
            }
            if (after_launch && !stateful)
                SPM_TRY((*after_launch)(H));
            SPM_HIP_CHECK(ctx, hipMemcpyAsync(c, H->d_count, kCntReadBack * sizeof(unsigned long long), hipMemcpyDeviceToHost, ctx->stream));
            SPM_HIP_CHECK(ctx, hipStreamSynchronize(ctx->stream));
            if (c[kCntVoid] == 0)
                ctx->band_dirty = false;
            scan_decision d = decide_scan(c, S.filt, H->cap, S.retry, attempt, A.tune.cand_cap);
            if (d.what == scan_outcome::more_room) {
                if (spm_trace_on())
                    fprintf(stderr, "[spm_hip] scan attempt %d starts over:%s%s%s (survivor slots drawn %llu of %llu, band slots %llu of %llu, "
                                    "overflow flags %llu, spans that gave up %llu)\n",
                            attempt, d.more_surv ? " survivor list too small" : "", d.more_bands ? " band list too small" : "",
                            d.more_seen ? " dedupe set too small" : "", c[kCntSurvSlots], (unsigned long long)H->cand_cap,
                            c[kCntBandSlots], (unsigned long long)H->band_cap, c[kCntVoid], c[kCntSpansGaveUp]);
                S.retry = d.next;
                ++attempt;
                SPM_TRY(clear_counters());
                continue;
            }
            take_stats(H, c);
            if (scan_clean(c, H->cand_cap))
                raise_hints(*ps, c);
            const bool rescan = d.what == scan_outcome::span_fallback;
            if (rescan) {
                SPM_TRY(span_fallback(c));
                d = decide_scan(c, S.filt, H->cap, S.retry, attempt, A.tune.cand_cap, true);
            }
            S.retry = d.next;
            switch (d.what) {
            case scan_outcome::brute_fallback:
                H->stats.fell_back = 1;
                use_filter = false;
                return clear_counters(false);
            case scan_outcome::with_seen:
            case scan_outcome::with_full_seen:
                SPM_TRY(clear_counters());
                ++round;
                attempt = 0;
                continue;
            case scan_outcome::final_hits:
            case scan_outcome::caller_overflow:
                H->n = c[kCntHits];
                H->counted = true;
                if (!rescan && d.what == scan_outcome::final_hits && after_launch && !stateful) {
                    H->hook_final = true;
                    H->fan_count = c[kCntFanOut];
                }
                return SPM_OK;
            case scan_outcome::more_room:
            case scan_outcome::span_fallback:
                return SPM_E_INVALID;
            }
        }
        return SPM_OK;
    }

    dev_scratch state_mem;
    uint32_t *d_in = nullptr, *d_out = nullptr;
    size_t st_words = 0;
    std::vector<uint32_t> h_in;
    int state_open()
    {
        if (!stateful)
            return SPM_OK;
        st_words = (size_t)ps->n_groups * (ps->is_myers() ? 2 * ps->NW + 1 : ps->NW) * 64;
        SPM_HIP_CHECK(ctx, state_mem.alloc(&d_in, st_words * 4 * 2));
        d_out = d_in + st_words;
        if (has_state) {
            state_to_internal(ps, state_in, h_in);
            SPM_HIP_CHECK(ctx, hipMemcpyAsync(d_in, h_in.data(), st_words * 4, hipMemcpyHostToDevice, ctx->stream));
        }
        return SPM_OK;
    }
    int state_close(bool have, bool aside)
    {
        if (state_out && !have) {
            SPM_TRY(run_brute(A, S, tail_begin, end, tail_begin, has_state && tail_begin == begin ? d_in : nullptr, d_out, false, true));
            H->stats.main_launches -= aside ? 1 : 0;
        }
        SPM_HIP_CHECK(ctx, hipEventRecord(H->ev[3], ctx->stream));
        std::vector<uint32_t> h_out(state_out ? st_words : 0);
        if (state_out)
            SPM_HIP_CHECK(ctx, hipMemcpyAsync(h_out.data(), d_out, st_words * 4, hipMemcpyDeviceToHost, ctx->stream));
        if (d_in)
            SPM_HIP_CHECK(ctx, hipStreamSynchronize(ctx->stream));
        if (state_out)
            state_from_internal(ps, h_out, state_out);
        return SPM_OK;
    }

    int stateful_remainder()
    {
        SPM_TRY(state_open());
        if (has_state) {
            SPM_TRY(run_brute(A, S, begin, begin + state_prefix, begin, d_in, nullptr, true, true));
            H->stats.main_launches--;
            H->counted = false;
        }
        return state_close(false, true);
    }

    int brute_engine()
    {
        H->stats.engine_used = SPM_ENGINE_BRUTE;
        SPM_TRY(state_open());
        SPM_HIP_CHECK(ctx, hipEventRecord(H->ev[1], ctx->stream));
        const uint64_t range = end - begin;
        const bool prefix = ps->algo == SPM_ALGO_MYERS_PREFIX;
        const uint64_t warm = ps->max_window > 0 ? ps->max_window - 1 : 0;
        const uint64_t pass_begin = begin - std::min(warm, begin - A.ctx_begin);
        const bool one_pass_state = state_out && (prefix || (range <= (1u << 16) && (has_state || pass_begin <= tail_begin)));
        SPM_TRY(host_segments());
        SPM_TRY(run_brute(A, S, begin, end, A.ctx_begin, has_state ? d_in : nullptr, one_pass_state ? d_out : nullptr, true,
                          one_pass_state));
        SPM_HIP_CHECK(ctx, hipEventRecord(H->ev[2], ctx->stream));
        return state_close(one_pass_state, false);
    }

    void trace(clk::time_point t_call) const
    {
        spm_scan_stats st{};
        spm_hip_hits_stats(H, &st);
        fprintf(stderr, "[spm_hip] scan [%llu, %llu)%s: engine %s%s, %u main launch(es); %.3f ms (main %.3f, verification %.3f); "
                        "%llu seed-checked pairs, %u bands, %llu hits%s; host %.3f ms\n",
                (unsigned long long)begin, (unsigned long long)end, segmented ? " segmented" : "",
                st.engine_used == SPM_ENGINE_FILTER ? (ps->filter_dense ? "filter (dense pass)" : "filter") : "brute",
                st.fell_back ? " after a whole-scan fallback" : "", st.main_launches, st.ms_total, st.ms_main, st.ms_verify,
                (unsigned long long)st.n_candidates, st.n_bands, (unsigned long long)st.n_hits,
                st.fallback_spans ? " (spans re-scanned by the brute-force kernel)" : "", ms_since(t_call));
    }
};

}

int scan_impl(spm_ctx *ctx, const spm_text *text, uint64_t begin, uint64_t end, const spm_patterns *patterns,
              const spm_scan_opts *opts_in, const void *state_in, void *state_out, const uint64_t *seg_offsets,
              uint64_t n_segments, spm_hits **out, const uint64_t *d_seg_offsets, const uint32_t *d_seg_owned,
              const std::function<int(spm_hits *)> *after_launch)
{
    if (!ctx || !text || !patterns || !out || begin > end || end > text->n) {
        SPM_SET_ERR(ctx, "spm_hip_scan: invalid argument");
        return SPM_E_INVALID;
    }
    if (patterns->sigma != text->sigma) {
        SPM_SET_ERR(ctx, "spm_hip_scan: text sigma %u != pattern sigma %u", text->sigma, patterns->sigma);
        return SPM_E_INVALID;
    }
    spm_scan_opts opts{};
    if (opts_in)
        opts = *opts_in;
    const auto t_call = clk::now();
    SPM_HIP_CHECK(ctx, hipSetDevice(ctx->device));

    std::unique_ptr<spm_hits, void (*)(spm_hits *)> H(new spm_hits, spm_hip_hits_destroy);
    H->ctx = ctx;
    H->cap = opts.max_hits ? opts.max_hits : (1ull << 20);
    SPM_TRY(acquire_hits(ctx, H.get()));
    H->al_text = text;
    H->al_patterns = patterns;
    H->al_lo = opts.left_context ? 0 : begin;
    H->al_pos_offset = opts.pos_offset;
    H->al_stateful = state_in != nullptr;
    H->al_device_segs = d_seg_offsets != nullptr && seg_offsets == nullptr;
    if (seg_offsets)
        H->al_segs.assign(seg_offsets, seg_offsets + n_segments + 1);

    const bool has_state = state_in != nullptr, stateful = has_state || state_out != nullptr;
    const bool segmented = seg_offsets || d_seg_offsets;
    const uint64_t state_prefix = has_state && patterns->max_window > 0 ? patterns->max_window - 1 : 0;
    bool use_filter = false;
    SPM_TRY(choose_engine(ctx, patterns, opts, end - begin, stateful, segmented, state_prefix, use_filter));
    const bool chunk = use_filter && has_state;
    const scan_args A{ctx, text, chunk ? begin + state_prefix : begin, end, chunk || !opts.left_context ? begin : 0, patterns, opts,
                      H.get(), scan_tuning::from_env(), seg_offsets, n_segments, d_seg_offsets, d_seg_owned};
    const uint64_t tail_len = 2ull * patterns->max_m + 4;
    const uint64_t tail_begin = std::max(has_state ? begin : A.ctx_begin, end > tail_len ? end - tail_len : 0);
    scan_call C{A, ctx, patterns, H.get(), begin, end, state_in, state_out, has_state, stateful, segmented, state_prefix, tail_begin,
                after_launch};
    C.S.segs = seg_offsets;

    SPM_HIP_CHECK(ctx, hipEventRecord(H->ev[0], ctx->stream));
    H->timed = true;
    const bool past_prefix_hits = patterns->algo == SPM_ALGO_MYERS_PREFIX && !stateful &&
                                  begin - A.ctx_begin >= patterns->max_window;
    if (patterns->n == 0 || past_prefix_hits || (end == begin && (has_state || !state_out || A.ctx_begin == begin))) {
        SPM_TRY(C.finish_trivial());
        *out = H.release();
        return SPM_OK;
    }
    if (use_filter) {
        H->stats.engine_used = SPM_ENGINE_FILTER;
        bool deferred = false;
        SPM_TRY(C.filter_attempts(use_filter, deferred));
        if (deferred) {
            *out = H.release();
            return SPM_OK;
        }
    }
    if (use_filter && stateful)
        SPM_TRY(C.stateful_remainder());
    if (!use_filter)
        SPM_TRY(C.brute_engine());
    if (spm_trace_on())
        C.trace(t_call);
    *out = H.release();
    return SPM_OK;
}


int spm_complete_deferred(spm_hits *h)
{
    if (!h->pending)
        return SPM_OK;
    spm_ctx *ctx = h->ctx;
    h->pending = false;
    if (!h->c_on_the_way) {
        SPM_HIP_CHECK(ctx, hipMemcpyAsync(h->h_c, h->d_count, kCntReadBack * sizeof(unsigned long long), hipMemcpyDeviceToHost, ctx->stream));
        SPM_HIP_CHECK(ctx, hipEventRecord(h->ev_done, ctx->stream));
        h->c_on_the_way = true;
    }
    SPM_HIP_CHECK(ctx, hipEventSynchronize(h->ev_done));
    const unsigned long long *c = h->h_c;
    take_stats(h, c);
    const bool clean = scan_clean(c, h->cand_cap);
    if (c[kCntVoid] != 0)
        ctx->band_dirty = true;
    if (clean || (c[kCntHits] > h->cap && c[kCntVoid] == 0)) {
        if (clean)
            raise_hints(*h->d_patterns, c);
        h->n = c[kCntHits];
        h->counted = true;
        return SPM_OK;
    }
    spm_scan_opts o = h->d_opts;
    o.flags &= ~SPM_SCAN_DEFER;
    spm_hits *again = nullptr;
    const int rc = scan_impl(ctx, h->d_text, h->d_begin, h->d_end, h->d_patterns, &o, nullptr, nullptr, nullptr, 0, &again);
    if (rc != SPM_OK)
        return rc;
    hits_adopt(*h, *again);
    spm_hip_hits_destroy(again);
    return SPM_OK;
}
```

### libspm_amd/csrc/scan_filter.hip

```cpp
#include "internal.hpp"
#include "filter.hpp"

namespace
{
template <typename K, typename... Args>
void launch(K kernel, dim3 grid, uint32_t threads, size_t lds, hipStream_t s, Args... args)
{
    hipFuncSetAttribute((const void *)kernel, hipFuncAttributeMaxDynamicSharedMemorySize, (int)lds);
    hipLaunchKernelGGL(kernel, grid, dim3(threads), lds, s, args...);
}

using filter_kernel = void (*)(filter_params);
using packed_kernel = void (*)(filter_params, const uint4 *);

template <int S, int U, bool KM>
filter_kernel sparse_kernel(uint32_t hv, uint32_t sigma)
{
    if (hv == 2 && sigma == 5)
        return seed_filter_kernel<S, U, 2, 5, KM>;
    if (hv == 2 && sigma == 15)
        return seed_filter_kernel<S, U, 2, 15, KM>;
    if (hv == 1 && sigma == 4)
        return seed_filter_kernel<S, U, 1, 4, KM>;
    if constexpr (S >= 4)
        if (hv == 2 && sigma == 4)
            return seed_filter_kernel<S, U, 2, 4, KM>;
    return nullptr;
}

filter_kernel select_filter_kernel(const filter_index &F, uint32_t sigma, bool km)
{
    if (F.dense) {
        switch (F.n_pat) {
        case 0:
        case 1: return seed_filter_dense_kernel<4, 1>;
        case 2: return seed_filter_dense_kernel<4, 2>;
        case 3: return seed_filter_dense_kernel<4, 3>;
        default: return nullptr;
        }
    }
    if (F.hash_variant == 4) {
        if (F.stride == 1)
            return km ? seed_filter_dense_kernel<4, 1, 1, true> : seed_filter_dense_kernel<4, 1, 1, false>;
        if (F.stride == 2)
            return km ? seed_filter_dense_kernel<4, 1, 2, true> : seed_filter_dense_kernel<4, 1, 2, false>;
        return nullptr;
    }
    switch (F.stride) {
    case 16: return km ? nullptr : sparse_kernel<16, 8, false>(F.hash_variant, sigma);
    case 8: return km ? nullptr : sparse_kernel<8, 8, false>(F.hash_variant, sigma);
    case 4: return km ? nullptr : sparse_kernel<4, 8, false>(F.hash_variant, sigma);
    case 2: return km ? sparse_kernel<2, 2, true>(F.hash_variant, sigma) : sparse_kernel<2, 2, false>(F.hash_variant, sigma);
    case 1:
        if (F.anchor_cm != 0 && F.hash_variant == 2 && sigma == 4 && !km)
            return seed_filter_kernel<1, 4, 2, 4, false, true>;
        return km ? sparse_kernel<1, 2, true>(F.hash_variant, sigma) : sparse_kernel<1, 2, false>(F.hash_variant, sigma);
    default: return nullptr;
    }
}

packed_kernel select_packed_kernel(uint32_t stride, bool km)
{
    if (km)
        return nullptr;
    switch (stride) {
    case 16: return seed_filter_packed_kernel<16, 4, 2, false>;
    case 8: return seed_filter_packed_kernel<8, 4, 2, false>;
    case 4: return seed_filter_packed_kernel<4, 2, 2, false>;
    default: return nullptr;
    }
}

template <int NWN>
void launch_verify_nw(const verify_params &V, dim3 grid, hipStream_t s)
{
    uint32_t threads = 256;
    const size_t per_thread = (size_t)(V.sigma + 1) * NWN * 4 + 2 * 16;
    while (threads > 64 && per_thread * threads > 128 * 1024)
        threads >>= 1;
    const size_t lds = per_thread * threads + (size_t)(threads / 64) * kHitStage * sizeof(spm_hit);
    launch(verify_kernel<NWN>, grid, threads, lds, s, V);
}

template <int G>
void launch_verify_wave_g(verify_params V, const uint32_t *peq_bot, uint32_t max_m, dim3 grid, hipStream_t s)
{
    grid.x *= 4;
    const uint32_t n_slots = 2 * V.max_k + 1 + V.max_span;
    V.wave_text = ((max_m + V.max_k + n_slots + 16 + 15) & ~15u) + 16;
    const size_t per_group = ((n_slots * 2 + 15) & ~15u) + V.wave_text;
    launch(verify_wave_kernel<G, 1>, grid, 64, (64 / G) * per_group, s, V, peq_bot);
}

void launch_verify_wave(uint32_t n_blocks, const verify_params &V, const uint32_t *peq_bot, uint32_t max_m, dim3 grid,
                        hipStream_t s)
{
    if (n_blocks <= 8)
        launch_verify_wave_g<8>(V, peq_bot, max_m, grid, s);
    else if (n_blocks <= 16)
        launch_verify_wave_g<16>(V, peq_bot, max_m, grid, s);
    else if (n_blocks <= 32)
        launch_verify_wave_g<32>(V, peq_bot, max_m, grid, s);
    else
        launch_verify_wave_g<64>(V, peq_bot, max_m, grid, s);
}

void launch_verify(uint32_t nwn, const verify_params &V, dim3 grid, hipStream_t s)
{
    switch (nwn) {
    case 1: launch_verify_nw<1>(V, grid, s); break;
    case 2: launch_verify_nw<2>(V, grid, s); break;
    case 3: launch_verify_nw<3>(V, grid, s); break;
    case 4: launch_verify_nw<4>(V, grid, s); break;
    case 5: launch_verify_nw<5>(V, grid, s); break;
    case 6: launch_verify_nw<6>(V, grid, s); break;
    case 7: launch_verify_nw<7>(V, grid, s); break;
    case 8: launch_verify_nw<8>(V, grid, s); break;
    case 16: launch_verify_nw<16>(V, grid, s); break;
    case 32: launch_verify_nw<32>(V, grid, s); break;
    default: launch_verify_nw<64>(V, grid, s); break;
    }
}

}

int ensure_band_table(spm_ctx *ctx, uint64_t slots)
{
    if (ctx->band_slots >= slots && !ctx->band_dirty)
        return SPM_OK;
    if (ctx->band_slots < slots) {
        const auto t0 = clk::now();
        if (ctx->d_band_tab) {
            SPM_HIP_CHECK(ctx, hipStreamSynchronize(ctx->stream));
            hipFree(ctx->d_band_tab);
            ctx->d_band_tab = nullptr;
            ctx->band_slots = 0;
        }
        SPM_HIP_CHECK(ctx, hipMalloc(&ctx->d_band_tab, slots * sizeof(ulonglong2)));
        ctx->band_slots = slots;
        if (spm_trace_on())
            fprintf(stderr, "[spm_hip] band table grows to %.1f MiB: %.2f ms\n", slots * sizeof(ulonglong2) / 1048576.0, ms_since(t0));
    }
    SPM_HIP_CHECK(ctx, hipMemsetAsync(ctx->d_band_tab, 0xFF, ctx->band_slots * sizeof(ulonglong2), ctx->stream));
    SPM_HIP_CHECK(ctx, hipMemsetAsync(ctx->d_table_poison, 0, 4, ctx->stream));
    ctx->band_dirty = false;
    return SPM_OK;
}

namespace
{
static_assert(sizeof(survivor) == kSurvivorBytes && sizeof(band_rec) == kBandRecBytes, "scan_plan.hpp sizes the lists");

struct filter_run
{
    const scan_args &A;
    const retry_state &retry;
    spm_ctx *ctx;
    const spm_patterns *ps;
    spm_hits *H;
    filter_sizes Z;
    survivor *surv = nullptr;
    unsigned long long *seen = nullptr;
    band_rec *bands = nullptr;
    uint64_t *ovf = nullptr;
    const uint64_t *d_seg = nullptr;
    uint64_t n_seg = 0;
    uint32_t seg_bits = 0;
    bool exact_hits = false, skip_seen = false;

    int lay_out()
    {
        SPM_TRY(ensure_scratch(ctx, Z.surv_bytes + Z.seen_bytes + Z.band_bytes + Z.ovf_bytes));
        exact_hits = ps->max_k == 0 && !Z.overlap && ps->filter_max_range == 0 && ps->d_ranks;
        if (exact_hits && ps->exact_whole < 0) {
            bool whole = true;
            for (uint32_t p = 0; p < ps->n && whole; ++p)
                whole = ps->seed_n[p] == 1 && ps->seed_q[p] == (uint32_t)ps->m[p];
            ps->exact_whole = whole ? 1 : 0;
        }
        exact_hits = exact_hits && ps->exact_whole == 1;
        if (!exact_hits)
            SPM_TRY(ensure_band_table(ctx, Z.band_slots));
        surv = (survivor *)ctx->d_scratch;
        seen = (unsigned long long *)((uint8_t *)surv + Z.surv_bytes);
        bands = (band_rec *)((uint8_t *)seen + Z.seen_bytes);
        ovf = (uint64_t *)((uint8_t *)bands + Z.band_bytes);
        skip_seen = exact_hits && !retry.need_seen;
        if (!skip_seen)
            SPM_HIP_CHECK(ctx, hipMemsetAsync(seen, 0xFF, Z.seen_bytes, ctx->stream));
        if (!exact_hits)
            ctx->band_dirty = true;
        return SPM_OK;
    }

    int launch_passes()
    {
        filter_params P{};
        P.text = A.text->d;
        P.text_alloc = A.text->owned ? A.text->alloc : A.text->n;
        const uint64_t reach = ps->max_window;
        P.lo = A.begin >= A.ctx_begin + reach ? A.begin - reach : A.ctx_begin;
        P.hi = A.end;
        P.surv = surv;
        P.counters = H->d_count;
        P.surv_cap = Z.surv_cap;
        P.ovf_spans = ovf;
        P.ovf_cap = kOvfCap;
        for (size_t fi = 0; fi < ps->fidx.size(); ++fi) {
            const filter_index &F = ps->fidx[fi];
            P.stride = F.stride;
            P.key_len = F.key_len;
            P.key_mask = F.key_len >= 16 ? 0xFFFFFFFFu : ((1u << (2 * F.key_len)) - 1);
            P.bitmap_words = F.hash_variant == 2 ? 1024 : F.bitmap_words;
            P.lds_words = F.lds_words;
            P.chd_slot_mask = F.chd_slot_mask;
            P.chd_bucket_shift = F.chd_bucket_shift;
            P.chd_disp_off = F.chd_disp_off;
            P.n_probes = F.n_probes;
            P.bitmap = F.d_bitmap;
            P.pass = (uint32_t)fi;
            P.anchor_c = F.anchor_c;
            P.anchor_cm = F.anchor_cm;
            P.n_pat = F.n_pat;
            for (uint32_t i = 0; i < kDensePatterns; ++i) {
                P.pat_c[i] = F.pat_c[i];
                P.pat_cm[i] = F.pat_cm[i];
            }
            P.bucket_shift = F.bucket_shift;
            P.buckets = reinterpret_cast<const uint4 *>(F.d_buckets);
            if (fi > 0)
                SPM_HIP_CHECK(ctx, hipMemsetAsync(H->d_count + kCntSpanHead, 0, sizeof(unsigned long long), ctx->stream));
            const bool km = F.key_len < 16;
            const bool bits = F.hash_variant == 4;
            const bool use_packed = F.hash_variant == 2 && A.text->d_packed && ps->sigma == 4 && F.stride >= 2 &&
                                    !(A.opts.flags & SPM_SCAN_IGNORE_PACKED);
            const bool wide_ok = use_packed || F.stride == 2 || (F.stride == 1 && !km && ps->sigma == 4);
            const uint32_t threads = (F.dense || bits || wide_ok) ? 1024 : 512;
            const size_t lds = (size_t)F.lds_words * 4 + 16 + 16 * kCandRec * 4 + ((F.dense || bits) ? 16 * sizeof(dense_queue) : 0);
            const uint32_t wg_per_cu = (uint32_t)std::max<size_t>(1, std::min<size_t>((160 * 1024) / lds, 2048 / threads));
            const uint32_t grid = ctx->n_cu * wg_per_cu;
            const uint64_t n_waves = (uint64_t)grid * (threads / 64);
            const uint64_t n_chunks = (P.hi - (P.lo & ~1023ull) + 1023) / 1024;
            uint64_t span = n_chunks / (n_waves * 32) + 1;
            if (span < 64)
                span = std::max<uint64_t>(span, std::min<uint64_t>(64, n_chunks / (n_waves * 4) + 1));
            span = std::min<uint64_t>(std::max<uint64_t>(span, 8), 4096);
            span = (span + 7) & ~7ull;
            P.span_chunks = (uint32_t)span;
            P.span_unit = 1024;
            const int sb = A.tune.span_budget;
            P.span_budget = sb > 0 ? (uint32_t)sb : (uint32_t)std::max<uint64_t>(256, span * 1024 / 4);
            P.dynamic = span >= 192 ? 1u : 2u;
            P.hash_variant = F.hash_variant;
            if (use_packed) {
                filter_params Q = P;
                const uint64_t n_pchunks = (Q.hi - (Q.lo & ~4095ull) + 4095) / 4096;
                uint64_t pspan = n_pchunks / (n_waves * 8) + 1;
                pspan = std::min<uint64_t>(std::max<uint64_t>(pspan, 4), 4096);
                pspan = (pspan + 3) & ~3ull;
                Q.span_chunks = (uint32_t)pspan;
                Q.span_unit = 4096;
                if (sb <= 0)
                    Q.span_budget = (uint32_t)std::max<uint64_t>(256, pspan * 4096 / 4);
                Q.dynamic = pspan >= 48 ? 1u : 2u;
                const packed_kernel k = select_packed_kernel(F.stride, km);
                if (!k) {
                    SPM_SET_ERR(ctx, "internal: no packed filter kernel for stride %u, key length %u", F.stride, F.key_len);
                    return SPM_E_UNSUPPORTED;
                }
                launch(k, dim3(grid), threads, lds, ctx->stream, Q, reinterpret_cast<const uint4 *>(A.text->d_packed));
            } else {
                const filter_kernel k = select_filter_kernel(F, ps->sigma, km);
                if (!k) {
                    SPM_SET_ERR(ctx, "internal: no filter kernel for stride %u, key length %u, sigma %u, hash variant %u, %u patterns",
                                F.stride, F.key_len, ps->sigma, F.hash_variant, F.n_pat);
                    return SPM_E_UNSUPPORTED;
                }
                launch(k, dim3(grid), threads, lds, ctx->stream, P);
            }
            SPM_HIP_CHECK(ctx, hipGetLastError());
            H->stats.main_launches++;
        }
        return SPM_OK;
    }

    template <typename Params>
    void fill_shared(Params &X) const
    {
        X.text = A.text->d;
        X.text_alloc = A.text->owned ? A.text->alloc : A.text->n;
        X.scan_begin = A.begin;
        X.scan_end = A.end;
        X.pos_offset = A.opts.pos_offset;
        X.counters = H->d_count;
        X.bands = bands;
        X.band_cap = Z.band_cap;
        X.band_tab = ctx->d_band_tab;
        X.table_mask = (uint32_t)(Z.band_slots - 1);
        X.band_bits = 43 - seg_bits;
        X.Bw = Z.Bw;
        X.overlap = Z.overlap ? 1u : 0u;
        X.max_m = ps->max_m;
        X.m = ps->d_m;
        X.k = ps->d_k;
        X.report_begin = ps->is_myers() ? 0 : 1;
        X.seen_mask = (uint32_t)(Z.seen_slots - 1);
        X.hits = H->d_hits;
        X.hit_counter = H->d_count + kCntHits;
        X.overflow = H->d_count + kCntVoid;
        X.hit_cap = H->cap;
        X.seg_offsets = d_seg;
        X.n_segments = n_seg;
        X.seg_owned = A.d_seg_owned;
    }

    int launch_resolve()
    {
        if (A.d_seg_offsets) {
            d_seg = A.d_seg_offsets;
            n_seg = A.n_segments;
        } else if (A.seg_offsets) {
            uint64_t *d = nullptr;
            SPM_HIP_CHECK(ctx, hipMalloc(&d, (A.n_segments + 1) * sizeof(uint64_t)));
            hipFree(H->d_aux[1]);
            H->d_aux[1] = d;
            SPM_HIP_CHECK(ctx, hipMemcpyAsync(d, A.seg_offsets, (A.n_segments + 1) * sizeof(uint64_t),
                                              hipMemcpyHostToDevice, ctx->stream));
            d_seg = d;
            n_seg = A.n_segments;
        }
        while (n_seg && (1ull << seg_bits) < n_seg + 1)
            ++seg_bits;
        resolve_params R{};
        fill_shared(R);
        R.surv = surv;
        R.surv_cap = Z.surv_cap;
        R.passes = ps->d_pass_tab;
        R.entries = ps->d_entries;
        R.key_len = ps->filter_key_len;
        R.needle_ranks = ps->d_ranks;
        R.needle_offsets = ps->d_offsets;
        R.seed_q = ps->d_seed_q;
        R.flank_check = (ps->sigma == 4 && !Z.overlap && R.needle_ranks) ? 1u : 0u;
        R.pieces_check = R.flank_check;
        R.hay_begin = A.ctx_begin;
        R.hay_end = A.end;
        R.needle_pk = ps->d_needle_pk;
        R.pk_offsets = ps->d_pk_offsets;
        R.exact_hits = exact_hits ? 1u : 0u;
        R.seen = skip_seen ? nullptr : seen;
        R.table_poison = ctx->d_table_poison;
        const uint64_t surv_expect = ps->cand_hint ? 2 * ps->cand_hint : Z.surv_cap;
        const uint64_t rmax = (uint64_t)ctx->n_cu * 5;
        const uint64_t per_wg = (surv_expect + 255) / 256 <= rmax ? 256 : 1024;
        const uint32_t rgrid = (uint32_t)std::min<uint64_t>(rmax, std::max<uint64_t>(ctx->n_cu / 2, (surv_expect + per_wg - 1) / per_wg));
        hipLaunchKernelGGL(resolve_kernel, dim3(rgrid), dim3(256), 0, ctx->stream, R);
        SPM_HIP_CHECK(ctx, hipGetLastError());
        return SPM_OK;
    }

    int launch_bands(bool runs)
    {
        verify_params V{};
        fill_shared(V);
        V.ctx_begin = A.ctx_begin;
        V.surplus = ps->d_surplus;
        V.peq32 = ps->d_peq_verify ? ps->d_peq_verify : ps->d_peq;
        V.sigma = ps->sigma;
        V.nw_table = ps->NW;
        V.max_k = ps->max_k;
        V.max_span = Z.max_span;
        V.seen = seen;
        V.band_counter = kCntBandSlots;
        band_rec *kept = bands + Z.band_cap;
        if (runs) {
            hipLaunchKernelGGL(band_runs_kernel, dim3(ctx->n_cu * 8), dim3(256), 0, ctx->stream, V, bands, kept, H->d_count + kCntRunHeads);
            SPM_HIP_CHECK(ctx, hipGetLastError());
            V.runs = 1;
            V.bands = kept;
            V.band_counter = kCntRunHeads;
        }
        if (Z.overlap) {
            hipLaunchKernelGGL(band_select_kernel, dim3(ctx->n_cu * 2), dim3(256), 0, ctx->stream, V, kept, H->d_count + kCntBandsSelected);
            SPM_HIP_CHECK(ctx, hipGetLastError());
            V.bands = kept;
            V.band_counter = kCntBandsSelected;
            V.preselected = 1;
        }
        if (exact_hits) {
        } else if (Z.use_wave) {
            launch_verify_wave(Z.nwn, V, ps->d_peq_bot, ps->max_m, dim3(ctx->n_cu * 16), ctx->stream);
        } else {
            const uint32_t nwn = Z.nwn > 8 ? ps->NW : Z.nwn;
            const uint64_t band_expect = ps->band_hint ? 2 * ps->band_hint : Z.band_cap;
            const uint32_t vgrid = (uint32_t)std::min<uint64_t>((uint64_t)ctx->n_cu * 4, std::max<uint64_t>(ctx->n_cu / 2, (band_expect + 255) / 256));
            launch_verify(nwn, V, dim3(vgrid), ctx->stream);
        }
        SPM_HIP_CHECK(ctx, hipGetLastError());
        if (runs) {
            hipLaunchKernelGGL(band_release_kernel, dim3(ctx->n_cu * 8), dim3(256), 0, ctx->stream, V, bands, (uint32_t)kCntBandSlots);
            SPM_HIP_CHECK(ctx, hipGetLastError());
        }
        return SPM_OK;
    }
};

}

int run_filter(const scan_args &A, const retry_state &R, filter_result &out)
{
    spm_ctx *ctx = A.ctx;
    spm_hits *H = A.hits;
    filter_run F{A, R, ctx, A.ps, H, size_filter(*A.ps, A.tune, A.end - A.begin, (uint64_t)ctx->n_cu, H->cap, R)};
    const filter_sizes &Z = F.Z;
    SPM_TRY(F.lay_out());
    const bool runs = !Z.overlap && !F.exact_hits && !Z.use_wave && Z.Bw <= 32 && !R.need_seen && A.tune.verify_runs != 0 &&
                      A.ps->band_hint >= (uint64_t)std::max(0, A.tune.verify_runs_min_bands);
    out = {F.seen, (uint32_t)(Z.seen_slots - 1), F.ovf, F.skip_seen || runs, Z.surv_cap, Z.band_cap};
    SPM_HIP_CHECK(ctx, hipEventRecord(H->ev[1], ctx->stream));
    SPM_TRY(F.launch_passes());
    SPM_HIP_CHECK(ctx, hipEventRecord(H->ev[2], ctx->stream));
    SPM_TRY(F.launch_resolve());
    SPM_TRY(F.launch_bands(runs));
    SPM_HIP_CHECK(ctx, hipEventRecord(H->ev[3], ctx->stream));
    return SPM_OK;
}


void spm_warm_filter_kernels()
{
    hipFuncAttributes a;
    (void)hipFuncGetAttributes(&a, (const void *)resolve_kernel);
}
```

### libspm_amd/csrc/scan_plan.hpp

```cpp
#pragma once

#include <algorithm>
#include <cmath>
#include <cstddef>
#include <utility>
#include <vector>

#include "hd.hpp"

namespace spm_hip
{

enum scan_counter : int
{
    kCntHits = 0,
    kCntSurvSlots = 1,
    kCntVoid = 2,
    kCntBandSlots = 3,
    kCntSpanHead = 4,
    kCntPairs = 5,
    kCntSpansGaveUp = 6,
    kCntBandsVerified = 7,
    kCntUnreadSurvSum = 8,
    kCntUnreadSurvMax = 9,
    kCntBandsSelected = 10,
    kCntRunHeads = 11,
    kCntFanOut = 12,
    kCntStateOnly = 13,
    kCntTicket = 15,
};
constexpr int kCntBlock = 16;
constexpr int kCntReadBack = 13;
constexpr int kCntReadBackRescan = 8;
constexpr int kCntReadBackCount = 4;
constexpr int kLandFanOut = 13;

SPM_HD inline bool scan_needs_host(const unsigned long long *c, unsigned long long cand_cap, const unsigned long long &n = 0,
                                   unsigned long long hit_cap = 0)
{
    return c[kCntVoid] != 0 || c[kCntSpansGaveUp] != 0 || c[kCntSurvSlots] > cand_cap || n > hit_cap;
}
SPM_HD inline bool scan_clean(const unsigned long long *c, unsigned long long cand_cap) { return !scan_needs_host(c, cand_cap); }

template <typename Set>
inline void raise_hints(const Set &ps, const unsigned long long *c)
{
    ps.cand_hint = std::max<uint64_t>(ps.cand_hint, c[kCntSurvSlots]);
    ps.hit_hint = std::max<uint64_t>(ps.hit_hint, c[kCntHits]);
    ps.band_hint = std::max<uint64_t>(ps.band_hint, c[kCntBandSlots]);
    ps.scanned = true;
}

struct retry_state
{
    uint64_t cand_cap_override = 0;
    uint64_t band_scale = 0;
    bool seen_full = false;
    bool need_seen = false;
};
struct filter_result
{
    unsigned long long *d_seen = nullptr;
    uint32_t seen_mask = 0;
    uint64_t *d_ovf = nullptr;
    bool seen_skipped = false;
    uint64_t cand_cap = 0, band_cap = 0;
};
enum class scan_outcome
{
    final_hits,
    caller_overflow,
    more_room,
    with_seen,
    with_full_seen,
    span_fallback,
    brute_fallback,
};
struct scan_decision
{
    scan_outcome what = scan_outcome::final_hits;
    retry_state next;
    bool more_surv = false, more_bands = false, more_seen = false;
};
constexpr uint64_t kSurvMax = 1ull << 27;
constexpr uint64_t kBandMax = 1ull << 28;

inline scan_decision decide_scan(const unsigned long long *c, const filter_result &ran, uint64_t hit_cap, const retry_state &rs,
                                 int attempt, int cand_cap_knob, bool rescanned = false)
{
    scan_decision d;
    d.next = rs;
    if (c[kCntHits] <= hit_cap && attempt < 2 && !rescanned) {
        d.more_surv = c[kCntSurvSlots] > ran.cand_cap && ran.cand_cap < kSurvMax && !cand_cap_knob;
        d.more_bands = c[kCntVoid] != 0 && c[kCntBandSlots] > ran.band_cap && ran.band_cap < kBandMax;
        d.more_seen = c[kCntVoid] != 0 && !rs.seen_full && !d.more_bands && c[kCntBandSlots] <= ran.band_cap;
        if (d.more_surv || d.more_bands || d.more_seen) {
            d.what = scan_outcome::more_room;
            if (d.more_surv)
                d.next.cand_cap_override = std::min<uint64_t>(
                    kSurvMax, std::max<uint64_t>(c[kCntSurvSlots] + c[kCntSurvSlots] / 8 + 4096, 4 * ran.cand_cap));
            if (d.more_bands)
                d.next.band_scale = std::max<uint64_t>(1, rs.band_scale) *
                                    std::max<uint64_t>(2, (c[kCntBandSlots] + ran.band_cap - 1) / ran.band_cap + 1);
            if (d.more_seen || c[kCntHits] > ((uint64_t)ran.seen_mask + 1) / 8)
                d.next.seen_full = true;
            return d;
        }
    }
    if (c[kCntHits] > hit_cap)
        d.what = scan_outcome::caller_overflow;
    else if (c[kCntVoid] != 0 && rescanned && !rs.seen_full) {
        d.what = scan_outcome::with_full_seen;
        d.next.seen_full = true;
    } else if (c[kCntVoid] != 0)
        d.what = scan_outcome::brute_fallback;
    else if (c[kCntSpansGaveUp] != 0 && !rescanned) {
        d.what = ran.seen_skipped ? scan_outcome::with_seen : scan_outcome::span_fallback;
        d.next.need_seen |= ran.seen_skipped;
    }
    return d;
}

inline void append_tiles(std::vector<uint64_t> &tab, uint64_t lo, uint64_t hi, uint64_t hay_lo, uint64_t warm, uint64_t tile)
{
    for (; lo < hi; lo += tile) {
        tab.push_back(lo >= hay_lo + warm ? lo - warm : hay_lo);
        tab.push_back(lo);
        tab.push_back(std::min(lo + tile, hi));
    }
}

constexpr uint64_t kOvfCap = 1ull << 17;

struct fallback_plan
{
    std::vector<std::pair<uint64_t, uint64_t>> ranges;
    uint64_t total = 0;
    uint64_t warm = 0, tile = 0;
};
inline fallback_plan plan_fallback(const uint64_t *ov, uint64_t n_ovf, uint64_t begin, uint64_t end, uint32_t max_window,
                                   uint64_t n_cu, uint32_t n_groups)
{
    fallback_plan F;
    std::vector<std::pair<uint64_t, uint64_t>> rg;
    rg.reserve(n_ovf);
    for (uint64_t i = 0; i < n_ovf; ++i) {
        const uint64_t b = ov[2 * i], len = ov[2 * i + 1];
        const uint64_t lo = std::max<uint64_t>(begin, b >= 16 ? b - 16 : 0);
        const uint64_t hi = std::min<uint64_t>(end, b + len + max_window);
        if (lo < hi)
            rg.emplace_back(lo, hi);
    }
    std::sort(rg.begin(), rg.end());
    for (const auto &r : rg) {
        if (!F.ranges.empty() && r.first <= F.ranges.back().second)
            F.ranges.back().second = std::max(F.ranges.back().second, r.second);
        else
            F.ranges.push_back(r);
    }
    for (const auto &r : F.ranges)
        F.total += r.second - r.first;
    F.warm = max_window > 0 ? max_window - 1 : 0;
    const uint64_t want_tiles = n_cu * 32 / std::max(1u, n_groups) + 1;
    F.tile = std::max<uint64_t>(std::max<uint64_t>(1024, (F.warm * 8 + 255) & ~255ull), (F.total / want_tiles + 255) & ~255ull);
    F.tile = std::min<uint64_t>(F.tile, 1u << 20);
    return F;
}
inline void fallback_tiles(const fallback_plan &F, uint64_t ctx_begin, const uint64_t *segs, uint64_t n_segments,
                           std::vector<uint64_t> &tab)
{
    for (const auto &r : F.ranges) {
        if (!segs) {
            append_tiles(tab, r.first, r.second, ctx_begin, F.warm, F.tile);
            continue;
        }
        uint64_t sidx = (uint64_t)(std::upper_bound(segs, segs + n_segments + 1, r.first) - segs);
        sidx = sidx ? sidx - 1 : 0;
        for (; sidx < n_segments && segs[sidx] < r.second; ++sidx)
            append_tiles(tab, std::max(r.first, segs[sidx]), std::min(r.second, segs[sidx + 1]), segs[sidx], F.warm, F.tile);
    }
}

constexpr uint32_t kChunkMin = 32;
constexpr size_t kSurvivorBytes = 16, kBandRecBytes = 16;

struct filter_sizes
{
    uint64_t surv_cap = 0, band_cap = 0, band_slots = 0, seen_slots = 0;
    uint32_t nwn = 1, Bw = 32, max_span = 31;
    bool use_wave = false;
    bool overlap = false;
    size_t surv_bytes = 0, seen_bytes = 0, band_bytes = 0, ovf_bytes = 0;
};

template <typename Set, typename Tune>
inline filter_sizes size_filter(const Set &ps, const Tune &tune, uint64_t symbols, uint64_t n_cu, uint64_t hit_cap, const retry_state &R)
{
    filter_sizes Z;
    const uint64_t kmax = ps.max_k;
    uint64_t est = std::max<uint64_t>(4096, 8ull * ps.n * (kmax + 1));
    est = std::max<uint64_t>(est, symbols / (ps.scanned ? 4096 : 2048));
    double chance = 0;
    for (const auto &F : ps.fidx)
        chance += (double)symbols / std::max(1u, F.stride) * (double)F.n_keys / std::pow(4.0, (double)F.key_len);
    est = std::max<uint64_t>(est, (uint64_t)(2.0 * chance));
    est = std::max<uint64_t>(est, ps.cand_hint + ps.cand_hint / 4);
    Z.surv_cap = std::min(2 * est + n_cu * 16 * kChunkMin, kSurvMax);
    if (R.cand_cap_override)
        Z.surv_cap = R.cand_cap_override;
    if (tune.cand_cap > 0)
        Z.surv_cap = (uint64_t)tune.cand_cap;
    const uint64_t band_want = std::max<uint64_t>(Z.surv_cap / 4, 2 * ps.band_hint);
    Z.band_cap = std::max<uint64_t>(band_want, 4096) * (R.band_scale ? R.band_scale : 1) + n_cu * 32 * kChunkMin;
    if (tune.band_cap > 0 && !R.band_scale)
        Z.band_cap = (uint64_t)tune.band_cap;
    Z.band_slots = 1u << 12;
    while (Z.band_slots < 2 * Z.band_cap)
        Z.band_slots <<= 1;
    Z.nwn = std::max(1u, (ps.max_m + 31) / 32);
    const int wave_min = tune.verify_wave_min_words;
    Z.use_wave = ps.d_peq_bot && wave_min > 0 && Z.nwn >= (uint32_t)wave_min && ps.sigma <= 5;
    Z.overlap = ps.d_surplus != nullptr;
    Z.Bw = 32;
    if (Z.overlap) {
        Z.Bw = (ps.max_k + 1) * (Z.use_wave ? 4 : 1);
        if (Z.Bw + ps.max_k > 2047)
            Z.Bw = ps.max_k + 1;
    }
    Z.max_span = Z.Bw - 1 + (Z.overlap ? ps.max_k + 1 : 0);
    uint64_t want_seen = std::min<uint64_t>(Z.band_cap * (2 * kmax + 1 + Z.max_span), std::max<uint64_t>(hit_cap, 1));
    if (!R.seen_full)
        want_seen = std::min<uint64_t>(want_seen, ps.scanned ? std::max<uint64_t>(1u << 18, 4 * ps.hit_hint) : (1ull << 22));
    Z.seen_slots = 1u << 16;
    while (Z.seen_slots < 2 * want_seen)
        Z.seen_slots <<= 1;
    Z.surv_bytes = Z.surv_cap * kSurvivorBytes;
    Z.seen_bytes = Z.seen_slots * sizeof(unsigned long long);
    Z.band_bytes = Z.band_cap * kBandRecBytes * 2;
    Z.ovf_bytes = kOvfCap * 2 * sizeof(uint64_t);
    return Z;
}

}
```

### libspm_amd/csrc/text.hip

```cpp
#include "internal.hpp"
#include "synth_kernels.hpp"
#include "text_kernels.hpp"

namespace spm_hip
{
thread_local std::string g_init_error;
}

extern "C" int spm_hip_init(int device, void *stream, spm_ctx **out)
{
    if (!out) {
        SPM_SET_ERR((spm_ctx *)nullptr, "spm_hip_init: out == NULL");
        return SPM_E_INVALID;
    }
    spm_ctx *none = nullptr;
    int n_dev = 0;
    SPM_HIP_CHECK(none, hipGetDeviceCount(&n_dev));
    if (device < 0 || device >= n_dev) {
        SPM_SET_ERR(none, "spm_hip_init: device %d not available (%d HIP devices)", device, n_dev);
        return SPM_E_INVALID;
    }
    SPM_HIP_CHECK(none, hipSetDevice(device));
    hipDeviceProp_t prop;
    SPM_HIP_CHECK(none, hipGetDeviceProperties(&prop, device));
    std::unique_ptr<spm_ctx> ctx(new spm_ctx);
    ctx->device = device;
    ctx->n_cu = prop.multiProcessorCount > 0 ? prop.multiProcessorCount : 256;
    if (stream) {
        ctx->stream = (hipStream_t)stream;
        ctx->own_stream = false;
    } else {
        SPM_HIP_CHECK(none, hipStreamCreateWithFlags(&ctx->stream, hipStreamNonBlocking));
        ctx->own_stream = true;
    }
    SPM_HIP_CHECK(none, hipHostMalloc(&ctx->h_counters, kCntBlock * sizeof(unsigned long long), hipHostMallocDefault));
    ctx->stage_half = (size_t)8 << 20;
    SPM_HIP_CHECK(none, hipHostMalloc(reinterpret_cast<void **>(&ctx->h_stage), 2 * ctx->stage_half, hipHostMallocDefault));
    for (int e = 0; e < 2; ++e)
        SPM_HIP_CHECK(none, hipEventCreateWithFlags(&ctx->stage_ev[e], hipEventDisableTiming));
    if (hipMalloc(&ctx->d_scratch, (size_t)128 << 20) == hipSuccess) {
        ctx->scratch_bytes = (size_t)128 << 20;
        memset(ctx->h_stage, 0, ctx->stage_half);
        (void)hipMemcpyAsync(ctx->d_scratch, ctx->h_stage, ctx->stage_half, hipMemcpyHostToDevice, ctx->stream);
        (void)hipEventRecord(ctx->stage_ev[0], ctx->stream);
        (void)hipMemcpyAsync(ctx->h_counters, ctx->d_scratch, kCntBlock * sizeof(unsigned long long), hipMemcpyDeviceToHost, ctx->stream);
        (void)hipStreamSynchronize(ctx->stream);
    } else {
        ctx->d_scratch = nullptr;
    }
    SPM_HIP_CHECK(none, hipMalloc(reinterpret_cast<void **>(&ctx->d_table_poison), 16));
    SPM_HIP_CHECK(none, hipMemsetAsync(ctx->d_table_poison, 0, 16, ctx->stream));
    {
        hits_block b;
        b.cap = 1ull << 20;
        bool ok = hipMalloc(&b.d_hits, b.cap * sizeof(spm_hit)) == hipSuccess &&
                  hipMalloc(&b.d_count, kCntBlock * sizeof(unsigned long long)) == hipSuccess;
        for (int e = 0; e < 4 && ok; ++e)
            ok = hipEventCreate(&b.ev[e]) == hipSuccess;
        if (ok && hipHostMalloc(reinterpret_cast<void **>(&b.h_c), kCntBlock * sizeof(unsigned long long), hipHostMallocDefault) != hipSuccess)
            b.h_c = nullptr;
        if (ok && hipEventCreateWithFlags(&b.ev_done, hipEventDisableTiming) != hipSuccess)
            b.ev_done = nullptr;
        if (ok && hipMemsetAsync(b.d_count, 0, kCntBlock * sizeof(unsigned long long), ctx->stream) == hipSuccess) {
            b.zeroed = true;
            ctx->pool.push_back(b);
        } else {
            hipFree(b.d_hits);
            hipFree(b.d_count);
            for (int e = 0; e < 4; ++e)
                if (b.ev[e])
                    hipEventDestroy(b.ev[e]);
            if (b.h_c)
                hipHostFree(b.h_c);
            if (b.ev_done)
                hipEventDestroy(b.ev_done);
        }
    }
    spm_warm_text_kernels();
    spm_warm_brute_kernels();
    spm_warm_filter_kernels();
    spm_warm_hits_kernels();
    spm_warm_jst_kernels();
    spm_warm_align_kernels();
    *out = ctx.release();
    return SPM_OK;
}

extern "C" void spm_hip_destroy(spm_ctx *ctx)
{
    if (!ctx)
        return;
    hipSetDevice(ctx->device);
    hipStreamSynchronize(ctx->stream);
    for (hits_block &b : ctx->pool) {
        hipFree(b.d_hits);
        hipFree(b.d_count);
        for (int e = 0; e < 4; ++e)
            if (b.ev[e])
                hipEventDestroy(b.ev[e]);
        if (b.h_c)
            hipHostFree(b.h_c);
        if (b.ev_done)
            hipEventDestroy(b.ev_done);
    }
    for (auto &b : ctx->jst_pool)
        hipFree(b.first);
    hipFree(ctx->d_table_poison);
    if (ctx->h_counters)
        hipHostFree(ctx->h_counters);
    if (ctx->h_stage)
        hipHostFree(ctx->h_stage);
    for (int e = 0; e < 2; ++e)
        if (ctx->stage_ev[e])
            hipEventDestroy(ctx->stage_ev[e]);
    if (ctx->own_stream)
        hipStreamDestroy(ctx->stream);
    hipFree(ctx->d_scratch);
    hipFree(ctx->d_band_tab);
    delete ctx;
}

extern "C" const char *spm_hip_last_error(const spm_ctx *ctx)
{
    return ctx ? ctx->err.c_str() : spm_hip::g_init_error.c_str();
}

extern "C" int spm_hip_synchronize(spm_ctx *ctx)
{
    if (!ctx)
        return SPM_E_INVALID;
    SPM_HIP_CHECK(ctx, hipStreamSynchronize(ctx->stream));
    return SPM_OK;
}

int text_alloc(spm_ctx *ctx, uint64_t n, uint32_t sigma, spm_text **out)
{
    std::unique_ptr<spm_text> t(new spm_text);
    t->ctx = ctx;
    t->n = n;
    t->sigma = sigma;
    t->alloc = ((n + 1023) & ~1023ull) + 1024;
    t->owned = true;
    SPM_HIP_CHECK(ctx, hipSetDevice(ctx->device));
    SPM_HIP_CHECK(ctx, hipMalloc(&t->d, t->alloc));
    *out = t.release();
    return SPM_OK;
}

extern "C" int spm_hip_text_upload(spm_ctx *ctx, const uint8_t *ranks, uint64_t n, uint32_t sigma, spm_text **out)
{
    if (!ctx || !out || (n && !ranks) || sigma < 2 || sigma > 255) {
        SPM_SET_ERR(ctx, "spm_hip_text_upload: invalid argument");
        return SPM_E_INVALID;
    }
    for (uint64_t i = 0; i < n; ++i)
        if (ranks[i] >= sigma) {
            SPM_SET_ERR(ctx, "spm_hip_text_upload: symbol %u at %llu is not a rank < sigma=%u", ranks[i],
                        (unsigned long long)i, sigma);
            return SPM_E_INVALID;
        }
    spm_text *t = nullptr;
    int rc = text_alloc(ctx, n, sigma, &t);
    if (rc != SPM_OK)
        return rc;
    if (n) {
        hipError_t e = hipMemcpyAsync(t->d, ranks, n, hipMemcpyHostToDevice, ctx->stream);
        if (e == hipSuccess)
            e = hipStreamSynchronize(ctx->stream);
        if (e != hipSuccess) {
            SPM_SET_ERR(ctx, "text upload failed: %s", hipGetErrorString(e));
            spm_hip_text_destroy(t);
            return SPM_E_HIP;
        }
    }
    *out = t;
    return SPM_OK;
}

extern "C" int spm_hip_text_wrap(spm_ctx *ctx, const void *device_ranks, uint64_t n, uint32_t sigma, spm_text **out)
{
    if (!ctx || !out || (n && !device_ranks) || ((uintptr_t)device_ranks & 15) || sigma < 2 || sigma > 255) {
        SPM_SET_ERR(ctx, "spm_hip_text_wrap: invalid argument (pointer must be 16-byte aligned)");
        return SPM_E_INVALID;
    }
    if (n) {
        SPM_HIP_CHECK(ctx, hipSetDevice(ctx->device));
        unsigned int *d_bad = nullptr;
        dev_scratch tmp;
        SPM_HIP_CHECK(ctx, tmp.alloc(&d_bad, sizeof(unsigned int)));
        SPM_HIP_CHECK(ctx, hipMemsetAsync(d_bad, 0, sizeof(unsigned int), ctx->stream));
        const uint64_t n_q = (n + 15) / 16;
        const uint32_t grid = (uint32_t)std::min<uint64_t>((n_q + 255) / 256, (uint64_t)ctx->n_cu * 16);
        hipLaunchKernelGGL(text_validate_kernel, dim3(grid), dim3(256), 0, ctx->stream, (const uint8_t *)device_ranks, n,
                           sigma, d_bad);
        SPM_HIP_CHECK(ctx, hipGetLastError());
        unsigned int bad = 0;
        SPM_HIP_CHECK(ctx, hipMemcpyAsync(&bad, d_bad, sizeof(bad), hipMemcpyDeviceToHost, ctx->stream));
        SPM_HIP_CHECK(ctx, hipStreamSynchronize(ctx->stream));
        if (bad) {
            SPM_SET_ERR(ctx, "spm_hip_text_wrap: the buffer holds symbols that are not ranks < sigma=%u", sigma);
            return SPM_E_INVALID;
        }
    }
    spm_text *t = new spm_text;
    t->ctx = ctx;
    t->d = (uint8_t *)device_ranks;
    t->n = n;
    t->alloc = n;
    t->sigma = sigma;
    t->owned = false;
    *out = t;
    return SPM_OK;
}

extern "C" int spm_hip_text_generate(spm_ctx *ctx, uint64_t seed, uint64_t global_begin, uint64_t n, spm_text **out)
{
    if (!ctx || !out || (global_begin & 31)) {
        SPM_SET_ERR(ctx, "spm_hip_text_generate: global_begin must be a multiple of 32");
        return SPM_E_INVALID;
    }
    spm_text *t = nullptr;
    int rc = text_alloc(ctx, n, 4, &t);
    if (rc != SPM_OK)
        return rc;
    if (n) {
        const uint64_t n_words = (n + 31) / 32;
        const uint32_t grid = (uint32_t)std::min<uint64_t>((n_words + 255) / 256, (uint64_t)ctx->n_cu * 16);
        hipLaunchKernelGGL(synth_text_kernel, dim3(grid), dim3(256), 0, ctx->stream, t->d, seed, global_begin, n);
        hipError_t e = hipGetLastError();
        if (e == hipSuccess)
            e = hipStreamSynchronize(ctx->stream);
        if (e != hipSuccess) {
            SPM_SET_ERR(ctx, "text generate failed: %s", hipGetErrorString(e));
            spm_hip_text_destroy(t);
            return SPM_E_HIP;
        }
    }
    *out = t;
    return SPM_OK;
}

extern "C" int spm_hip_text_generate_repeats(spm_ctx *ctx, uint64_t seed, uint64_t global_begin, uint64_t n,
                                             uint32_t repeat_ppm, spm_text **out)
{
    if (!ctx || !out || (global_begin & 31) || repeat_ppm > 130000) {
        SPM_SET_ERR(ctx, "spm_hip_text_generate_repeats: global_begin must be a multiple of 32, repeat_ppm <= 130000");
        return SPM_E_INVALID;
    }
    spm_text *t = nullptr;
    int rc = text_alloc(ctx, n, 4, &t);
    if (rc != SPM_OK)
        return rc;
    if (n) {
        const uint64_t n_q = (n + 15) / 16;
        const uint32_t grid = (uint32_t)std::min<uint64_t>((n_q + 255) / 256, (uint64_t)ctx->n_cu * 32);
        hipLaunchKernelGGL(synth_repeat_text_kernel, dim3(grid), dim3(256), 0, ctx->stream, t->d, seed, repeat_ppm,
                           global_begin, n);
        hipError_t e = hipGetLastError();
        if (e == hipSuccess)
            e = hipStreamSynchronize(ctx->stream);
        if (e != hipSuccess) {
            SPM_SET_ERR(ctx, "text generate failed: %s", hipGetErrorString(e));
            spm_hip_text_destroy(t);
            return SPM_E_HIP;
        }
    }
    *out = t;
    return SPM_OK;
}

extern "C" int spm_hip_text_pack(spm_ctx *ctx, spm_text *text)
{
    if (!ctx || !text) {
        SPM_SET_ERR(ctx, "spm_hip_text_pack: invalid argument");
        return SPM_E_INVALID;
    }
    if (text->sigma != 4) {
        SPM_SET_ERR(ctx, "spm_hip_text_pack: only dna4 haystacks have a 2-bit encoding (sigma = %u)", text->sigma);
        return SPM_E_INVALID;
    }
    if (text->d_packed)
        return SPM_OK;
    SPM_HIP_CHECK(ctx, hipSetDevice(ctx->device));
    const uint64_t n_words = (text->n + 15) / 16;
    const uint64_t padded = ((text->n + 4095) / 4096) * 256 + 2048;
    uint32_t *d = nullptr;
    unsigned int *d_bad = nullptr;
    SPM_HIP_CHECK(ctx, hipMalloc(&d, padded * sizeof(uint32_t)));
    SPM_HIP_CHECK(ctx, hipMalloc(&d_bad, sizeof(unsigned int)));
    SPM_HIP_CHECK(ctx, hipMemsetAsync(d, 0, padded * sizeof(uint32_t), ctx->stream));
    SPM_HIP_CHECK(ctx, hipMemsetAsync(d_bad, 0, sizeof(unsigned int), ctx->stream));
    if (n_words) {
        const uint32_t grid = (uint32_t)std::min<uint64_t>((n_words + 255) / 256, (uint64_t)ctx->n_cu * 16);
        hipLaunchKernelGGL(text_pack_kernel, dim3(grid), dim3(256), 0, ctx->stream, text->d,
                           text->owned ? std::min(text->alloc, text->n) : text->n, d, n_words, d_bad);
        SPM_HIP_CHECK(ctx, hipGetLastError());
    }
    unsigned int bad = 0;
    SPM_HIP_CHECK(ctx, hipMemcpyAsync(&bad, d_bad, sizeof(bad), hipMemcpyDeviceToHost, ctx->stream));
    SPM_HIP_CHECK(ctx, hipStreamSynchronize(ctx->stream));
    hipFree(d_bad);
    if (bad) {
        hipFree(d);
        SPM_SET_ERR(ctx, "spm_hip_text_pack: the text holds symbols that are not dna4 ranks (>= 4)");
        return SPM_E_INVALID;
    }
    text->d_packed = d;
    text->packed_words = padded;
    return SPM_OK;
}

extern "C" int spm_hip_text_is_packed(const spm_text *text) { return text && text->d_packed ? 1 : 0; }

extern "C" int spm_hip_text_download(spm_ctx *ctx, const spm_text *text, uint64_t begin, uint64_t n, uint8_t *dst)
{
    if (!ctx || !text || begin + n > text->n || (n && !dst)) {
        SPM_SET_ERR(ctx, "spm_hip_text_download: invalid argument");
        return SPM_E_INVALID;
    }
    if (n) {
        SPM_HIP_CHECK(ctx, hipMemcpyAsync(dst, text->d + begin, n, hipMemcpyDeviceToHost, ctx->stream));
        SPM_HIP_CHECK(ctx, hipStreamSynchronize(ctx->stream));
    }
    return SPM_OK;
}

extern "C" uint64_t spm_hip_text_length(const spm_text *t) { return t ? t->n : 0; }
extern "C" const void *spm_hip_text_device_ptr(const spm_text *t) { return t ? t->d : nullptr; }

extern "C" void spm_hip_text_destroy(spm_text *t)
{
    if (!t)
        return;
    if (t->owned)
        hipFree(t->d);
    hipFree(t->d_packed);
    delete t;
}

extern "C" uint64_t spm_hip_synth_pattern(uint64_t seed_text, uint64_t seed_pat, uint64_t n_total, uint32_t p,
                                          uint32_t L, uint32_t kmax, uint8_t *out)
{
    return synth_pattern(seed_text, seed_pat, n_total, p, L, kmax, out);
}

extern "C" uint64_t spm_hip_synth_repeat_pattern(uint64_t seed_text, uint64_t seed_pat, uint64_t n_total, uint32_t p,
                                                 uint32_t L, uint32_t kmax, uint32_t repeat_ppm, uint32_t across_every,
                                                 uint8_t *out)
{
    return synth_repeat_pattern(seed_text, seed_pat, n_total, p, L, kmax, repeat_ppm, across_every, out);
}

extern "C" void spm_hip_synth_repeat_text(uint64_t seed, uint32_t repeat_ppm, uint64_t begin, uint64_t n, uint8_t *out)
{
    for (uint64_t i = 0; i < n; ++i)
        out[i] = repeat_base(seed, repeat_ppm, begin + i);
}

extern "C" uint64_t spm_hip_mix64(uint64_t z) { return mix64(z); }

extern "C" const char *spm_hip_version(void) { return "libspm_hip 0.2 (gfx950)"; }

void spm_warm_text_kernels()
{
    hipFuncAttributes a;
    (void)hipFuncGetAttributes(&a, (const void *)synth_text_kernel);
}
```

Baseline: 6507.

## Run deferred filter passes on a second stream with double-buffered survivor slots

Adds a secondary 'lane' stream on which the filter passes of deferred scans are launched, so a scan's filter can overlap the previous scan's resolve and verify stages on the main stream. Survivor and overflow buffers move from the shared scratch into two rotating slots, with events tracking when each slot has been read and when hit-counter blocks were cleared. Verify launches shrink their workgroups when streaming filter kernels hold LDS, so the two can co-reside on a CU. This adds event bookkeeping, extra memory and a global live-context registry, and only applies when SPM_SCAN_DEFER is set and the stream is not being captured.

After: 6692, median of 6. +2.8%, better.

```diff
diff --git a/libspm_amd/csrc/common.hpp b/libspm_amd/csrc/common.hpp
--- a/libspm_amd/csrc/common.hpp
+++ b/libspm_amd/csrc/common.hpp
@@ -12,6 +12,7 @@
 
 #include "../../include/spm_hip.h"
 #include "scan_plan.hpp"
+#include "scan_lanes.hpp"
 
 namespace spm_hip
 {
@@ -36,6 +37,8 @@
     bool zeroed = false;
     unsigned long long *h_c = nullptr;
     hipEvent_t ev_done = nullptr;
+    hipEvent_t ev_clear = nullptr;
+    uint64_t clear_ticket = 0;
 };
 
 struct spm_ctx
@@ -47,6 +50,13 @@
     std::string err;
     void *d_scratch = nullptr;
     size_t scratch_bytes = 0;
+    hipStream_t lane = nullptr;
+    hipEvent_t lane_ev = nullptr;
+    hipEvent_t slot_ev[spm_hip::kSurvSlots] = {nullptr, nullptr};
+    void *d_slot[spm_hip::kSurvSlots] = {nullptr, nullptr};
+    size_t slot_bytes[spm_hip::kSurvSlots] = {0, 0};
+    spm_hip::lane_book lanes;
+    size_t lds_streaming_max = 0;
     std::vector<hits_block> pool;
     std::vector<std::pair<void *, uint64_t>> jst_pool;
     ulonglong2 *d_band_tab = nullptr;
diff --git a/libspm_amd/csrc/filter.hpp b/libspm_amd/csrc/filter.hpp
--- a/libspm_amd/csrc/filter.hpp
+++ b/libspm_amd/csrc/filter.hpp
@@ -1322,10 +1322,11 @@
     queue_sync();
 }
 
-__global__ __launch_bounds__(256) void resolve_kernel(const resolve_params R)
-{
-    __shared__ pair_queue pair_queues[4];
-    __shared__ band_queue band_queues[4];
+template <int WAVES>
+__global__ __launch_bounds__(WAVES * 64) void resolve_kernel(const resolve_params R)
+{
+    __shared__ pair_queue pair_queues[WAVES];
+    __shared__ band_queue band_queues[WAVES];
     unsigned long long n = R.counters[kCntSurvSlots];
     if (blockIdx.x == 0 && threadIdx.x == 0) {
         atomicAdd(&R.counters[kCntUnreadSurvSum], n);
diff --git a/libspm_amd/csrc/hits.hip b/libspm_amd/csrc/hits.hip
--- a/libspm_amd/csrc/hits.hip
+++ b/libspm_amd/csrc/hits.hip
@@ -161,6 +161,7 @@
         SPM_HIP_CHECK(h->ctx, hipEventRecord(h->ev_done, h->ctx->stream));
         h->c_on_the_way = true;
         h->d_count_cleared = true;
+        SPM_TRY(note_cleared(h->ctx, *h));
     }
     return SPM_OK;
 }
@@ -204,17 +205,18 @@
         (void)spm_complete_deferred(h);
     if (h->d_aux[0] || h->d_aux[1]) {
         if (h->ctx)
-            hipStreamSynchronize(h->ctx->stream);
+            (void)drain_queues(h->ctx);
         hipFree(h->d_aux[0]);
         hipFree(h->d_aux[1]);
     }
     if (h->ctx && h->d_hits && h->d_count && h->ev[3] && h->ctx->pool.size() < 8) {
         hits_block b = *h;
-        b.zeroed = h->d_count_cleared || hipMemsetAsync(b.d_count, 0, kCntBlock * sizeof(unsigned long long), h->ctx->stream) == hipSuccess;
+        b.zeroed = h->d_count_cleared || (hipMemsetAsync(b.d_count, 0, kCntBlock * sizeof(unsigned long long), h->ctx->stream) == hipSuccess &&
+                                          note_cleared(h->ctx, b) == SPM_OK);
         h->ctx->pool.push_back(b);
     } else {
         if (h->ctx)
-            hipStreamSynchronize(h->ctx->stream);
+            (void)drain_queues(h->ctx);
         hipFree(h->d_hits);
         hipFree(h->d_count);
         for (int i = 0; i < 4; ++i)
@@ -224,6 +226,8 @@
             hipHostFree(h->h_c);
         if (h->ev_done)
             hipEventDestroy(h->ev_done);
+        if (h->ev_clear)
+            hipEventDestroy(h->ev_clear);
     }
     delete h;
 }
diff --git a/libspm_amd/csrc/internal.hpp b/libspm_amd/csrc/internal.hpp
--- a/libspm_amd/csrc/internal.hpp
+++ b/libspm_amd/csrc/internal.hpp
@@ -115,9 +115,14 @@
 void state_from_internal(const spm_patterns *p, const std::vector<uint32_t> &in, void *state);
 int text_alloc(spm_ctx *ctx, uint64_t n, uint32_t sigma, spm_text **out);
 int ensure_scratch(spm_ctx *ctx, size_t bytes);
+int ensure_slot(spm_ctx *ctx, int slot, size_t bytes);
+int drain_queues(spm_ctx *ctx);
+void drain_owner(spm_ctx *ctx);
+int open_lane(spm_ctx *ctx);
+int note_cleared(spm_ctx *ctx, hits_block &b);
 int run_brute(const scan_args &A, const scan_state &S, uint64_t begin, uint64_t end, uint64_t ctx_begin,
               const uint32_t *d_state_in, uint32_t *d_state_out, bool report, bool single_tile);
-int run_filter(const scan_args &A, const retry_state &R, filter_result &out);
+int run_filter(const scan_args &A, const retry_state &R, filter_result &out, bool deferred);
 int scan_impl(spm_ctx *ctx, const spm_text *text, uint64_t begin, uint64_t end, const spm_patterns *patterns,
               const spm_scan_opts *opts_in, const void *state_in, void *state_out, const uint64_t *seg_offsets,
               uint64_t n_segments, spm_hits **out, const uint64_t *d_seg_offsets = nullptr,
diff --git a/libspm_amd/csrc/patterns.hip b/libspm_amd/csrc/patterns.hip
--- a/libspm_amd/csrc/patterns.hip
+++ b/libspm_amd/csrc/patterns.hip
@@ -234,6 +234,7 @@
 {
     if (!p)
         return;
+    drain_owner(p->ctx);
     hipFree(p->d_arena);
     hipFree(p->d_align);
     delete p;
diff --git a/libspm_amd/csrc/scan.hip b/libspm_amd/csrc/scan.hip
--- a/libspm_amd/csrc/scan.hip
+++ b/libspm_amd/csrc/scan.hip
@@ -1,27 +1,73 @@
 #include "internal.hpp"
 #include "filter_shared.hpp"
 
-int ensure_scratch(spm_ctx *ctx, size_t bytes)
-{
-    if (ctx->scratch_bytes >= bytes)
+namespace
+{
+int grow_buffer(spm_ctx *ctx, void *&d, size_t &have, size_t bytes, const char *what)
+{
+    if (have >= bytes)
         return SPM_OK;
     const auto t0 = clk::now();
-    if (ctx->d_scratch) {
-        SPM_HIP_CHECK(ctx, hipStreamSynchronize(ctx->stream));
-        SPM_HIP_CHECK(ctx, hipFree(ctx->d_scratch));
-        ctx->d_scratch = nullptr;
-        ctx->scratch_bytes = 0;
+    if (d) {
+        SPM_TRY(drain_queues(ctx));
+        SPM_HIP_CHECK(ctx, hipFree(d));
+        d = nullptr;
+        have = 0;
     }
     size_t want = bytes + bytes / 4;
-    hipError_t e = hipMalloc(&ctx->d_scratch, want);
+    hipError_t e = hipMalloc(&d, want);
     if (e != hipSuccess) {
         (void)hipGetLastError();
         want = bytes;
-        SPM_HIP_CHECK(ctx, hipMalloc(&ctx->d_scratch, want));
-    }
-    ctx->scratch_bytes = want;
+        SPM_HIP_CHECK(ctx, hipMalloc(&d, want));
+    }
+    have = want;
     if (spm_trace_on())
-        fprintf(stderr, "[spm_hip] scratch (survivor / band lists, dedupe set) grows to %.1f MiB: %.2f ms\n", want / 1048576.0, ms_since(t0));
+        fprintf(stderr, "[spm_hip] %s grows to %.1f MiB: %.2f ms\n", what, want / 1048576.0, ms_since(t0));
+    return SPM_OK;
+}
+}
+
+int drain_queues(spm_ctx *ctx)
+{
+    if (ctx->lane)
+        SPM_HIP_CHECK(ctx, hipStreamSynchronize(ctx->lane));
+    SPM_HIP_CHECK(ctx, hipStreamSynchronize(ctx->stream));
+    return SPM_OK;
+}
+
+int ensure_scratch(spm_ctx *ctx, size_t bytes)
+{
+    return grow_buffer(ctx, ctx->d_scratch, ctx->scratch_bytes, bytes, "scratch (band lists, dedupe set)");
+}
+
+int ensure_slot(spm_ctx *ctx, int slot, size_t bytes)
+{
+    return grow_buffer(ctx, ctx->d_slot[slot], ctx->slot_bytes[slot], bytes, "a survivor slot (survivor list, overflow spans)");
+}
+
+int open_lane(spm_ctx *ctx)
+{
+    if (!ctx->lane) {
+        SPM_HIP_CHECK(ctx, hipStreamCreateWithFlags(&ctx->lane, hipStreamNonBlocking));
+        SPM_HIP_CHECK(ctx, hipEventCreateWithFlags(&ctx->lane_ev, hipEventDisableTiming));
+        for (int s = 0; s < kSurvSlots; ++s)
+            SPM_HIP_CHECK(ctx, hipEventCreateWithFlags(&ctx->slot_ev[s], hipEventDisableTiming));
+    }
+    SPM_HIP_CHECK(ctx, hipEventRecord(ctx->lane_ev, ctx->stream));
+    SPM_HIP_CHECK(ctx, hipStreamWaitEvent(ctx->lane, ctx->lane_ev, 0));
+    return SPM_OK;
+}
+
+int note_cleared(spm_ctx *ctx, hits_block &b)
+{
+    b.clear_ticket = 0;
+    if (!ctx->lanes.lane_open)
+        return SPM_OK;
+    if (!b.ev_clear)
+        SPM_HIP_CHECK(ctx, hipEventCreateWithFlags(&b.ev_clear, hipEventDisableTiming));
+    SPM_HIP_CHECK(ctx, hipEventRecord(b.ev_clear, ctx->stream));
+    b.clear_ticket = note_block_cleared(ctx->lanes);
     return SPM_OK;
 }
 
@@ -61,8 +107,10 @@
         if (ctx->pool[i].cap == H->cap) {
             static_cast<hits_block &>(*H) = ctx->pool[i];
             ctx->pool.erase(ctx->pool.begin() + i);
-            if (!H->zeroed)
+            if (!H->zeroed) {
                 SPM_HIP_CHECK(ctx, hipMemsetAsync(H->d_count, 0, kCntBlock * sizeof(unsigned long long), ctx->stream));
+                SPM_TRY(note_cleared(ctx, *H));
+            }
             return SPM_OK;
         }
     const auto ta = clk::now();
@@ -73,7 +121,7 @@
     for (int i = 0; i < 4; ++i)
         SPM_HIP_CHECK(ctx, hipEventCreate(&H->ev[i]));
     SPM_HIP_CHECK(ctx, hipMemsetAsync(H->d_count, 0, kCntBlock * sizeof(unsigned long long), ctx->stream));
-    return SPM_OK;
+    return note_cleared(ctx, *H);
 }
 
 int choose_engine(spm_ctx *ctx, const spm_patterns *patterns, const spm_scan_opts &opts, uint64_t range, bool stateful,
@@ -171,6 +219,8 @@
         const uint64_t n_ovf = c[kCntSpansGaveUp];
         std::vector<uint64_t> ov(2 * n_ovf);
         SPM_HIP_CHECK(ctx, hipMemcpyAsync(ov.data(), S.filt.d_ovf, ov.size() * sizeof(uint64_t), hipMemcpyDeviceToHost, ctx->stream));
+        if (note_slot_read(ctx->lanes, S.filt.slot))
+            SPM_HIP_CHECK(ctx, hipEventRecord(ctx->slot_ev[S.filt.slot], ctx->stream));
         SPM_HIP_CHECK(ctx, hipStreamSynchronize(ctx->stream));
         const fallback_plan F = plan_fallback(ov.data(), n_ovf, A.begin, end, ps->max_window, (uint64_t)ctx->n_cu, ps->n_groups);
         if (segmented)
@@ -199,11 +249,13 @@
     int filter_attempts(bool &use_filter, bool &deferred)
     {
         unsigned long long *c = ctx->h_counters;
+        const bool may_defer = (A.opts.flags & SPM_SCAN_DEFER) && !stateful && !segmented && !after_launch;
         for (int round = 0, attempt = 0; round < 3;) {
-            SPM_TRY(run_filter(A, S.retry, S.filt));
+            const bool defer_now = may_defer && round == 0 && attempt == 0;
+            SPM_TRY(run_filter(A, S.retry, S.filt, defer_now));
             H->cand_cap = S.filt.cand_cap;
             H->band_cap = S.filt.band_cap;
-            if ((A.opts.flags & SPM_SCAN_DEFER) && round == 0 && attempt == 0 && !stateful && !segmented && !after_launch) {
+            if (defer_now) {
                 deferred = true;
                 return defer_completion();
             }
diff --git a/libspm_amd/csrc/scan_filter.hip b/libspm_amd/csrc/scan_filter.hip
--- a/libspm_amd/csrc/scan_filter.hip
+++ b/libspm_amd/csrc/scan_filter.hip
@@ -71,15 +71,20 @@
     }
 }
 
+constexpr size_t kCuLds = 160 * 1024;
+constexpr size_t kResolveLds4 = 4 * (sizeof(pair_queue) + sizeof(band_queue));
+
 template <int NWN>
-void launch_verify_nw(const verify_params &V, dim3 grid, hipStream_t s)
+void launch_verify_nw(const verify_params &V, dim3 grid, hipStream_t s, size_t lds_room)
 {
     uint32_t threads = 256;
     const size_t per_thread = (size_t)(V.sigma + 1) * NWN * 4 + 2 * 16;
     while (threads > 64 && per_thread * threads > 128 * 1024)
         threads >>= 1;
-    const size_t lds = per_thread * threads + (size_t)(threads / 64) * kHitStage * sizeof(spm_hit);
-    launch(verify_kernel<NWN>, grid, threads, lds, s, V);
+    const auto lds_of = [&](uint32_t t) { return per_thread * t + (size_t)(t / 64) * kHitStage * sizeof(spm_hit); };
+    for (; lds_room && threads > 64 && lds_of(threads) > lds_room; threads >>= 1)
+        grid.x *= 2;
+    launch(verify_kernel<NWN>, grid, threads, lds_of(threads), s, V);
 }
 
 template <int G>
@@ -105,20 +110,20 @@
         launch_verify_wave_g<64>(V, peq_bot, max_m, grid, s);
 }
 
-void launch_verify(uint32_t nwn, const verify_params &V, dim3 grid, hipStream_t s)
+void launch_verify(uint32_t nwn, const verify_params &V, dim3 grid, hipStream_t s, size_t lds_room)
 {
     switch (nwn) {
-    case 1: launch_verify_nw<1>(V, grid, s); break;
-    case 2: launch_verify_nw<2>(V, grid, s); break;
-    case 3: launch_verify_nw<3>(V, grid, s); break;
-    case 4: launch_verify_nw<4>(V, grid, s); break;
-    case 5: launch_verify_nw<5>(V, grid, s); break;
-    case 6: launch_verify_nw<6>(V, grid, s); break;
-    case 7: launch_verify_nw<7>(V, grid, s); break;
-    case 8: launch_verify_nw<8>(V, grid, s); break;
-    case 16: launch_verify_nw<16>(V, grid, s); break;
-    case 32: launch_verify_nw<32>(V, grid, s); break;
-    default: launch_verify_nw<64>(V, grid, s); break;
+    case 1: launch_verify_nw<1>(V, grid, s, lds_room); break;
+    case 2: launch_verify_nw<2>(V, grid, s, lds_room); break;
+    case 3: launch_verify_nw<3>(V, grid, s, lds_room); break;
+    case 4: launch_verify_nw<4>(V, grid, s, lds_room); break;
+    case 5: launch_verify_nw<5>(V, grid, s, lds_room); break;
+    case 6: launch_verify_nw<6>(V, grid, s, lds_room); break;
+    case 7: launch_verify_nw<7>(V, grid, s, lds_room); break;
+    case 8: launch_verify_nw<8>(V, grid, s, lds_room); break;
+    case 16: launch_verify_nw<16>(V, grid, s, lds_room); break;
+    case 32: launch_verify_nw<32>(V, grid, s, lds_room); break;
+    default: launch_verify_nw<64>(V, grid, s, lds_room); break;
     }
 }
 
@@ -131,7 +136,7 @@
     if (ctx->band_slots < slots) {
         const auto t0 = clk::now();
         if (ctx->d_band_tab) {
-            SPM_HIP_CHECK(ctx, hipStreamSynchronize(ctx->stream));
+            SPM_TRY(drain_queues(ctx));
             hipFree(ctx->d_band_tab);
             ctx->d_band_tab = nullptr;
             ctx->band_slots = 0;
@@ -167,10 +172,21 @@
     uint64_t n_seg = 0;
     uint32_t seg_bits = 0;
     bool exact_hits = false, skip_seen = false;
+    lane_plan L;
+    size_t lds_streaming = 0;
+
+    size_t lds_room() const
+    {
+        const size_t held = std::max(lds_streaming, ctx->lds_streaming_max);
+        return L.on_lane && held < kCuLds ? kCuLds - held : 0;
+    }
 
     int lay_out()
     {
-        SPM_TRY(ensure_scratch(ctx, Z.surv_bytes + Z.seen_bytes + Z.band_bytes + Z.ovf_bytes));
+        SPM_TRY(ensure_scratch(ctx, Z.seen_bytes + Z.band_bytes));
+        for (int s = 0; s < kSurvSlots; ++s)
+            if (s == L.slot || ctx->lanes.lane_open)
+                SPM_TRY(ensure_slot(ctx, s, Z.ovf_bytes + Z.surv_bytes));
         exact_hits = ps->max_k == 0 && !Z.overlap && ps->filter_max_range == 0 && ps->d_ranks;
         if (exact_hits && ps->exact_whole < 0) {
             bool whole = true;
@@ -181,10 +197,10 @@
         exact_hits = exact_hits && ps->exact_whole == 1;
         if (!exact_hits)
             SPM_TRY(ensure_band_table(ctx, Z.band_slots));
-        surv = (survivor *)ctx->d_scratch;
-        seen = (unsigned long long *)((uint8_t *)surv + Z.surv_bytes);
+        seen = (unsigned long long *)ctx->d_scratch;
         bands = (band_rec *)((uint8_t *)seen + Z.seen_bytes);
-        ovf = (uint64_t *)((uint8_t *)bands + Z.band_bytes);
+        ovf = (uint64_t *)ctx->d_slot[L.slot];
+        surv = (survivor *)((uint8_t *)ovf + Z.ovf_bytes);
         skip_seen = exact_hits && !retry.need_seen;
         if (!skip_seen)
             SPM_HIP_CHECK(ctx, hipMemsetAsync(seen, 0xFF, Z.seen_bytes, ctx->stream));
@@ -193,7 +209,7 @@
         return SPM_OK;
     }
 
-    int launch_passes()
+    int launch_passes(hipStream_t sq)
     {
         filter_params P{};
         P.text = A.text->d;
@@ -229,7 +245,7 @@
             P.bucket_shift = F.bucket_shift;
             P.buckets = reinterpret_cast<const uint4 *>(F.d_buckets);
             if (fi > 0)
-                SPM_HIP_CHECK(ctx, hipMemsetAsync(H->d_count + kCntSpanHead, 0, sizeof(unsigned long long), ctx->stream));
+                SPM_HIP_CHECK(ctx, hipMemsetAsync(H->d_count + kCntSpanHead, 0, sizeof(unsigned long long), sq));
             const bool km = F.key_len < 16;
             const bool bits = F.hash_variant == 4;
             const bool use_packed = F.hash_variant == 2 && A.text->d_packed && ps->sigma == 4 && F.stride >= 2 &&
@@ -239,6 +255,8 @@
             const size_t lds = (size_t)F.lds_words * 4 + 16 + 16 * kCandRec * 4 + ((F.dense || bits) ? 16 * sizeof(dense_queue) : 0);
             const uint32_t wg_per_cu = (uint32_t)std::max<size_t>(1, std::min<size_t>((160 * 1024) / lds, 2048 / threads));
             const uint32_t grid = ctx->n_cu * wg_per_cu;
+            lds_streaming = std::max(lds_streaming, (size_t)wg_per_cu * lds);
+            ctx->lds_streaming_max = std::max(ctx->lds_streaming_max, lds_streaming);
             const uint64_t n_waves = (uint64_t)grid * (threads / 64);
             const uint64_t n_chunks = (P.hi - (P.lo & ~1023ull) + 1023) / 1024;
             uint64_t span = n_chunks / (n_waves * 32) + 1;
@@ -268,7 +286,7 @@
                     SPM_SET_ERR(ctx, "internal: no packed filter kernel for stride %u, key length %u", F.stride, F.key_len);
                     return SPM_E_UNSUPPORTED;
                 }
-                launch(k, dim3(grid), threads, lds, ctx->stream, Q, reinterpret_cast<const uint4 *>(A.text->d_packed));
+                launch(k, dim3(grid), threads, lds, sq, Q, reinterpret_cast<const uint4 *>(A.text->d_packed));
             } else {
                 const filter_kernel k = select_filter_kernel(F, ps->sigma, km);
                 if (!k) {
@@ -276,7 +294,7 @@
                                 F.stride, F.key_len, ps->sigma, F.hash_variant, F.n_pat);
                     return SPM_E_UNSUPPORTED;
                 }
-                launch(k, dim3(grid), threads, lds, ctx->stream, P);
+                launch(k, dim3(grid), threads, lds, sq, P);
             }
             SPM_HIP_CHECK(ctx, hipGetLastError());
             H->stats.main_launches++;
@@ -354,8 +372,13 @@
         const uint64_t rmax = (uint64_t)ctx->n_cu * 5;
         const uint64_t per_wg = (surv_expect + 255) / 256 <= rmax ? 256 : 1024;
         const uint32_t rgrid = (uint32_t)std::min<uint64_t>(rmax, std::max<uint64_t>(ctx->n_cu / 2, (surv_expect + per_wg - 1) / per_wg));
-        hipLaunchKernelGGL(resolve_kernel, dim3(rgrid), dim3(256), 0, ctx->stream, R);
+        if (lds_room() && kResolveLds4 > lds_room())
+            hipLaunchKernelGGL(resolve_kernel<1>, dim3(rgrid * 4), dim3(64), 0, ctx->stream, R);
+        else
+            hipLaunchKernelGGL(resolve_kernel<4>, dim3(rgrid), dim3(256), 0, ctx->stream, R);
         SPM_HIP_CHECK(ctx, hipGetLastError());
+        if (note_slot_read(ctx->lanes, L.slot))
+            SPM_HIP_CHECK(ctx, hipEventRecord(ctx->slot_ev[L.slot], ctx->stream));
         return SPM_OK;
     }
 
@@ -394,7 +417,7 @@
             const uint32_t nwn = Z.nwn > 8 ? ps->NW : Z.nwn;
             const uint64_t band_expect = ps->band_hint ? 2 * ps->band_hint : Z.band_cap;
             const uint32_t vgrid = (uint32_t)std::min<uint64_t>((uint64_t)ctx->n_cu * 4, std::max<uint64_t>(ctx->n_cu / 2, (band_expect + 255) / 256));
-            launch_verify(nwn, V, dim3(vgrid), ctx->stream);
+            launch_verify(nwn, V, dim3(vgrid), ctx->stream, lds_room());
         }
         SPM_HIP_CHECK(ctx, hipGetLastError());
         if (runs) {
@@ -407,19 +430,52 @@
 
 }
 
-int run_filter(const scan_args &A, const retry_state &R, filter_result &out)
+int run_filter(const scan_args &A, const retry_state &R, filter_result &out, bool deferred)
 {
     spm_ctx *ctx = A.ctx;
     spm_hits *H = A.hits;
     filter_run F{A, R, ctx, A.ps, H, size_filter(*A.ps, A.tune, A.end - A.begin, (uint64_t)ctx->n_cu, H->cap, R)};
     const filter_sizes &Z = F.Z;
+    hipStreamCaptureStatus capture = hipStreamCaptureStatusNone;
+    if (deferred)
+        SPM_HIP_CHECK(ctx, hipStreamIsCapturing(ctx->stream, &capture));
+    const lane_plan &L = F.L = plan_lane(ctx->lanes, deferred, capture != hipStreamCaptureStatusNone, H->clear_ticket);
+    if (L.open_lane) {
+        const int rc = open_lane(ctx);
+        if (rc != SPM_OK) {
+            lane_failed_to_open(ctx->lanes, L);
+            return rc;
+        }
+    }
     SPM_TRY(F.lay_out());
     const bool runs = !Z.overlap && !F.exact_hits && !Z.use_wave && Z.Bw <= 32 && !R.need_seen && A.tune.verify_runs != 0 &&
                       A.ps->band_hint >= (uint64_t)std::max(0, A.tune.verify_runs_min_bands);
-    out = {F.seen, (uint32_t)(Z.seen_slots - 1), F.ovf, F.skip_seen || runs, Z.surv_cap, Z.band_cap};
-    SPM_HIP_CHECK(ctx, hipEventRecord(H->ev[1], ctx->stream));
-    SPM_TRY(F.launch_passes());
-    SPM_HIP_CHECK(ctx, hipEventRecord(H->ev[2], ctx->stream));
+    out = {F.seen, (uint32_t)(Z.seen_slots - 1), F.ovf, L.slot, F.skip_seen || runs, Z.surv_cap, Z.band_cap};
+    if (L.on_lane) {
+        int rc = SPM_OK;
+        const auto lane_part = [&]() -> int {
+            SPM_HIP_CHECK(ctx, hipEventRecord(H->ev[0], ctx->lane));
+            if (L.lane_wait_slot)
+                SPM_HIP_CHECK(ctx, hipStreamWaitEvent(ctx->lane, ctx->slot_ev[L.slot], 0));
+            if (L.lane_wait_clear)
+                SPM_HIP_CHECK(ctx, hipStreamWaitEvent(ctx->lane, H->ev_clear, 0));
+            SPM_HIP_CHECK(ctx, hipEventRecord(H->ev[1], ctx->lane));
+            SPM_TRY(F.launch_passes(ctx->lane));
+            SPM_HIP_CHECK(ctx, hipEventRecord(H->ev[2], ctx->lane));
+            SPM_HIP_CHECK(ctx, hipEventRecord(ctx->lane_ev, ctx->lane));
+            return SPM_OK;
+        };
+        if ((rc = lane_part()) != SPM_OK) {
+            (void)hipStreamSynchronize(ctx->lane);
+            return rc;
+        }
+        note_streamed(ctx->lanes);
+        SPM_HIP_CHECK(ctx, hipStreamWaitEvent(ctx->stream, ctx->lane_ev, 0));
+    } else {
+        SPM_HIP_CHECK(ctx, hipEventRecord(H->ev[1], ctx->stream));
+        SPM_TRY(F.launch_passes(ctx->stream));
+        SPM_HIP_CHECK(ctx, hipEventRecord(H->ev[2], ctx->stream));
+    }
     SPM_TRY(F.launch_resolve());
     SPM_TRY(F.launch_bands(runs));
     SPM_HIP_CHECK(ctx, hipEventRecord(H->ev[3], ctx->stream));
@@ -430,5 +486,5 @@
 void spm_warm_filter_kernels()
 {
     hipFuncAttributes a;
-    (void)hipFuncGetAttributes(&a, (const void *)resolve_kernel);
-}
+    (void)hipFuncGetAttributes(&a, (const void *)resolve_kernel<4>);
+}
diff --git a/libspm_amd/csrc/scan_lanes.hpp b/libspm_amd/csrc/scan_lanes.hpp
--- /dev/null
+++ b/libspm_amd/csrc/scan_lanes.hpp
@@ -0,0 +1,72 @@
+#pragma once
+
+#include <cstdint>
+
+namespace spm_hip
+{
+
+constexpr int kSurvSlots = 2;
+
+struct lane_book
+{
+    uint64_t recorded = 0;
+    uint64_t slot_reader[kSurvSlots] = {0, 0};
+    uint64_t lane_tail = 0;
+    int next_slot = 0;
+    bool lane_open = false;
+};
+
+struct lane_plan
+{
+    bool on_lane = false;
+    bool open_lane = false;
+    int slot = 0;
+    uint64_t lane_wait_slot = 0;
+    uint64_t lane_wait_clear = 0;
+    uint64_t lane_wait_open = 0;
+};
+
+inline lane_plan plan_lane(lane_book &B, bool deferred, bool capturing, uint64_t block_clear)
+{
+    lane_plan P;
+    P.on_lane = deferred && !capturing;
+    if (P.on_lane) {
+        P.slot = B.next_slot;
+        B.next_slot = (B.next_slot + 1) % kSurvSlots;
+        if (!B.lane_open) {
+            B.lane_open = P.open_lane = true;
+            P.lane_wait_open = ++B.recorded;
+        } else {
+            P.lane_wait_slot = B.slot_reader[P.slot];
+            P.lane_wait_clear = block_clear;
+        }
+        return P;
+    }
+    P.slot = 0;
+    return P;
+}
+
+inline void lane_failed_to_open(lane_book &B, const lane_plan &P)
+{
+    if (P.open_lane) {
+        B.lane_open = false;
+        B.next_slot = P.slot;
+    }
+}
+
+inline uint64_t note_streamed(lane_book &B)
+{
+    B.lane_tail = ++B.recorded;
+    return B.lane_tail;
+}
+
+inline uint64_t note_slot_read(lane_book &B, int slot)
+{
+    if (!B.lane_open)
+        return 0;
+    return B.slot_reader[slot] = ++B.recorded;
+}
+
+inline uint64_t note_block_cleared(lane_book &B) { return ++B.recorded; }
+
+}
diff --git a/libspm_amd/csrc/scan_plan.hpp b/libspm_amd/csrc/scan_plan.hpp
--- a/libspm_amd/csrc/scan_plan.hpp
+++ b/libspm_amd/csrc/scan_plan.hpp
@@ -63,6 +63,7 @@
     unsigned long long *d_seen = nullptr;
     uint32_t seen_mask = 0;
     uint64_t *d_ovf = nullptr;
+    int slot = 0;
     bool seen_skipped = false;
     uint64_t cand_cap = 0, band_cap = 0;
 };
diff --git a/libspm_amd/csrc/text.hip b/libspm_amd/csrc/text.hip
--- a/libspm_amd/csrc/text.hip
+++ b/libspm_amd/csrc/text.hip
@@ -2,9 +2,24 @@
 #include "synth_kernels.hpp"
 #include "text_kernels.hpp"
 
+#include <mutex>
+
 namespace spm_hip
 {
 thread_local std::string g_init_error;
+}
+
+namespace
+{
+std::mutex g_live_mutex;
+std::vector<spm_ctx *> g_live;
+}
+
+void drain_owner(spm_ctx *ctx)
+{
+    std::lock_guard<std::mutex> lock(g_live_mutex);
+    if (std::find(g_live.begin(), g_live.end(), ctx) != g_live.end())
+        (void)drain_queues(ctx);
 }
 
 extern "C" int spm_hip_init(int device, void *stream, spm_ctx **out)
@@ -38,6 +53,10 @@
     SPM_HIP_CHECK(none, hipHostMalloc(reinterpret_cast<void **>(&ctx->h_stage), 2 * ctx->stage_half, hipHostMallocDefault));
     for (int e = 0; e < 2; ++e)
         SPM_HIP_CHECK(none, hipEventCreateWithFlags(&ctx->stage_ev[e], hipEventDisableTiming));
+    if (hipMalloc(&ctx->d_slot[0], (size_t)32 << 20) == hipSuccess)
+        ctx->slot_bytes[0] = (size_t)32 << 20;
+    else
+        ctx->d_slot[0] = nullptr;
     if (hipMalloc(&ctx->d_scratch, (size_t)128 << 20) == hipSuccess) {
         ctx->scratch_bytes = (size_t)128 << 20;
         memset(ctx->h_stage, 0, ctx->stage_half);
@@ -82,6 +101,10 @@
     spm_warm_hits_kernels();
     spm_warm_jst_kernels();
     spm_warm_align_kernels();
+    {
+        std::lock_guard<std::mutex> lock(g_live_mutex);
+        g_live.push_back(ctx.get());
+    }
     *out = ctx.release();
     return SPM_OK;
 }
@@ -90,9 +113,23 @@
 {
     if (!ctx)
         return;
+    {
+        std::lock_guard<std::mutex> lock(g_live_mutex);
+        g_live.erase(std::remove(g_live.begin(), g_live.end(), ctx), g_live.end());
+    }
     hipSetDevice(ctx->device);
-    hipStreamSynchronize(ctx->stream);
+    (void)drain_queues(ctx);
+    if (ctx->lane) {
+        hipStreamDestroy(ctx->lane);
+        hipEventDestroy(ctx->lane_ev);
+        for (int s = 0; s < kSurvSlots; ++s)
+            hipEventDestroy(ctx->slot_ev[s]);
+    }
+    for (int s = 0; s < kSurvSlots; ++s)
+        hipFree(ctx->d_slot[s]);
     for (hits_block &b : ctx->pool) {
+        if (b.ev_clear)
+            hipEventDestroy(b.ev_clear);
         hipFree(b.d_hits);
         hipFree(b.d_count);
         for (int e = 0; e < 4; ++e)
@@ -129,8 +166,7 @@
 {
     if (!ctx)
         return SPM_E_INVALID;
-    SPM_HIP_CHECK(ctx, hipStreamSynchronize(ctx->stream));
-    return SPM_OK;
+    return drain_queues(ctx);
 }
 
 int text_alloc(spm_ctx *ctx, uint64_t n, uint32_t sigma, spm_text **out)
@@ -332,6 +368,7 @@
 {
     if (!t)
         return;
+    drain_owner(t->ctx);
     if (t->owned)
         hipFree(t->d);
     hipFree(t->d_packed);
```
